# jeremiahfaith/strainer2

Measured on AMD Instinct MI355X. Metric: metagenome bases/sec scanned at k=31, higher is better.
Workload: dtype u64

## Files before the change

strainer2_amd/csrc/sk_dev_kernels.hip.h:

```cpp

__constant__ signed char sk_comp_dev[256];

struct sk_wide_view {
    const char     *keys31;
    const uint32_t *rows;
    const uint32_t *index;
    uint32_t        wmask;
    uint32_t        nwide;
};

template <bool TALLY, bool UNION = false>
__global__ __launch_bounds__(256)
void sk_scan_wide(const uint8_t *__restrict__ stream, uint64_t nbytes, uint64_t emit_begin,
                  sk_table_view table, sk_wide_view wide, sk_sink sink,
                  const uint32_t *__restrict__ flags, uint32_t *__restrict__ next_flags)
{
    if (blockIdx.x == 0u && threadIdx.x < 4u) next_flags[threadIdx.x] = 0u;
    if (flags[0] == 0u) return;
    const uint32_t nodd = flags[2];
    const bool listed = nodd <= table.oddcap;
    const uint64_t nitems = listed ? (uint64_t)nodd * 46u : nbytes;
    const uint64_t stride = (uint64_t)gridDim.x * blockDim.x;
    for (uint64_t item = (uint64_t)blockIdx.x * blockDim.x + threadIdx.x; item < nitems; item += stride) {
        uint64_t p, owner = ~0ull;
        if (listed) { owner = table.oddlist[item / 46u]; p = owner * 16u + item % 46u; }
        else p = item;
        if (p < emit_begin || p >= nbytes || p < (uint64_t)(SK_K - 1)) continue;
        const uint8_t *w = stream + (p - (SK_K - 1));
        char u[SK_K];
        bool hard = false, pure = true;
        int last_odd = -1;
        for (int i = 0; i < SK_K; i++) {
            const uint32_t b = w[i];
            hard |= (bool)sk_is_hard_break(b);
            if (!sk_is_acgt(b)) { pure = false; last_odd = i; }
            u[i] = (char)sk_upper(b);
        }
        if (hard || pure) continue;
        if (listed && ((p - (SK_K - 1) + (uint64_t)last_odd) >> 4) != owner) continue;
        int sign = 0;
        for (int i = 0; i < SK_K && sign == 0; i++) {
            const signed char f = (signed char)u[i];
            const signed char r = sk_comp_dev[(uint8_t)u[SK_K - 1 - i]];
            sign = (f > r) - (r > f);
        }
        char o[SK_K + 1];
        if (sign >= 0) { for (int i = 0; i < SK_K; i++) o[i] = u[i]; }
        else           { for (int i = 0; i < SK_K; i++) o[SK_K - 1 - i] = (char)sk_comp_dev[(uint8_t)u[i]]; }
        o[SK_K] = 0;
        bool opure = true, has_n = false, has_nul = false;
        for (int i = 0; i < SK_K; i++) {
            opure &= (bool)sk_is_acgt((uint8_t)o[i]) & ((uint8_t)o[i] < 'a');
            has_n |= (o[i] == 'N');
            has_nul |= (o[i] == 0);
        }
        if (has_n || has_nul) continue;
        if (opure) {
            uint64_t key = 0;
            for (int i = 0; i < SK_K; i++) key = (key << 2) | sk_code((uint8_t)o[i]);
            sk_probe<TALLY, false, UNION>(key, table, sink, (uint32_t)p);
        } else if (wide.nwide) {
            uint32_t slot = sk_hash_wide(o) & wide.wmask;
            for (;;) {
                const uint32_t e = wide.index[slot];
                if (e == 0u) break;
                const char *cand = wide.keys31 + (size_t)(e - 1u) * 32u;
                bool same = true;
                for (int i = 0; i < SK_K; i++) same &= (cand[i] == o[i]);
                if (same) { sk_on_hit<TALLY, false, UNION>(sink, wide.rows[e - 1u], (uint32_t)p); break; }
                slot = (slot + 1u) & wide.wmask;
            }
        }
    }
}

__global__ void sk_fill64(uint64_t *p, uint64_t n, uint64_t v)
{
    const uint64_t stride = (uint64_t)gridDim.x * blockDim.x;
    for (uint64_t i = (uint64_t)blockIdx.x * blockDim.x + threadIdx.x; i < n; i += stride) p[i] = v;
}

__global__ void sk_table_insert(const uint64_t *__restrict__ in, uint32_t n, sk_u4 *slots, uint32_t mask, uint32_t *flags,
                                const uint32_t *__restrict__ perm, const uint32_t *__restrict__ locality)
{
    const uint32_t i = blockIdx.x * blockDim.x + threadIdx.x;
    if (i >= n) return;
    const uint64_t k = in[i];
    const uint32_t idx = perm ? perm[i] : i;
    if (k == SK_EMPTY64) return;
    if (k > SK_KMASK62) { atomicAdd(&flags[1], 1u); return; }
    uint32_t slot = sk_slot0(sk_khash(k), mask);
    for (;;) {
        const unsigned long long old = atomicCAS((unsigned long long *)&slots[slot],
                                                (unsigned long long)SK_EMPTY64, (unsigned long long)k);
        if (old == SK_EMPTY64) {
            ((uint32_t *)&slots[slot])[2] = idx;
            ((uint32_t *)&slots[slot])[3] = 0xFFFFFFFEu | (locality ? locality[i] >> 31 : 0u);
            return;
        }
        if (old == k) { atomicAdd(&flags[1], 1u); return; }
        slot = (slot + 1u) & mask;
    }
}

__global__ void sk_tally_compact(const uint32_t *__restrict__ tally, uint32_t nrec, uint32_t *__restrict__ out, unsigned long long *n)
{
    const uint32_t r = blockIdx.x * blockDim.x + threadIdx.x;
    const uint2 t = r < nrec ? ((const uint2 *)tally)[r] : make_uint2(0u, 0u);
    const unsigned long long m = __ballot(t.x != 0u);
    if (!m) return;
    const uint32_t lane = threadIdx.x & 63u, leader = (uint32_t)__builtin_ctzll(m);
    unsigned long long base = 0;
    if (lane == leader) base = atomicAdd(n, (unsigned long long)__popcll(m));
    base = ((unsigned long long)(uint32_t)__shfl((int)(uint32_t)(base >> 32), (int)leader) << 32) | (uint32_t)__shfl((int)(uint32_t)base, (int)leader);
    if (t.x != 0u) {
        uint32_t *o = out + 3ull * (base + (unsigned long long)__popcll(m & ((1ull << lane) - 1ull)));
        o[0] = r; o[1] = t.x; o[2] = t.y;
    }
}

__global__ void sk_inf_bitmap(const uint32_t *__restrict__ type, uint32_t n, uint32_t value, uint32_t *__restrict__ bits)
{
    const uint32_t i = blockIdx.x * blockDim.x + threadIdx.x;
    const bool is = i < n && type[i] == value;
    const unsigned long long m = __ballot(is);
    if ((threadIdx.x & 63u) == 0u && i < n + 64u) { bits[2u * (i >> 6)] = (uint32_t)m; bits[2u * (i >> 6) + 1u] = (uint32_t)(m >> 32); }
}

__global__ void sk_table_setpos(sk_u4 *slots, uint64_t nslots, const uint32_t *__restrict__ pos_by_idx)
{
    const uint64_t stride = (uint64_t)gridDim.x * blockDim.x;
    for (uint64_t i = (uint64_t)blockIdx.x * blockDim.x + threadIdx.x; i < nslots; i += stride) {
        const sk_u4 e = slots[i];
        if (sk_slot_key(e) == SK_EMPTY64) continue;
        ((uint32_t *)&slots[i])[3] = (pos_by_idx[e.z] << 1) | (e.w & 1u);
    }
}

#define SK_DIFF_PER_BLOCK 4096u
__global__ __launch_bounds__(256) void sk_diff_block_sums(const uint32_t *__restrict__ diff, uint32_t n, uint32_t *__restrict__ sums)
{
    __shared__ uint32_t part[256];
    const uint32_t base = blockIdx.x * SK_DIFF_PER_BLOCK + threadIdx.x * 16u;
    uint32_t t = 0;
    for (uint32_t i = 0; i < 16u; i++) if (base + i < n) t += diff[base + i];
    part[threadIdx.x] = t;
    __syncthreads();
    for (uint32_t d = 128u; d > 0u; d >>= 1) { if (threadIdx.x < d) part[threadIdx.x] += part[threadIdx.x + d]; __syncthreads(); }
    if (threadIdx.x == 0) sums[blockIdx.x] = part[0];
}
__global__ __launch_bounds__(1024) void sk_diff_scan_sums(uint32_t *sums, uint32_t nb)
{
    __shared__ uint32_t part[1024];
    const uint32_t per = (nb + 1023u) / 1024u, lo = threadIdx.x * per;
    uint32_t t = 0;
    for (uint32_t i = lo; i < lo + per && i < nb; i++) t += sums[i];
    part[threadIdx.x] = t;
    __syncthreads();
    for (uint32_t d = 1u; d < 1024u; d <<= 1) {
        const uint32_t v = threadIdx.x >= d ? part[threadIdx.x - d] : 0u;
        __syncthreads();
        part[threadIdx.x] += v;
        __syncthreads();
    }
    uint32_t run = part[threadIdx.x] - t;
    for (uint32_t i = lo; i < lo + per && i < nb; i++) { const uint32_t v = sums[i]; sums[i] = run; run += v; }
}
__global__ __launch_bounds__(256) void sk_diff_apply(uint32_t *__restrict__ diff, uint32_t n, const uint32_t *__restrict__ sums,
                                                      uint32_t *__restrict__ counts, uint32_t nrows)
{
    __shared__ uint32_t part[256];
    const uint32_t base = blockIdx.x * SK_DIFF_PER_BLOCK + threadIdx.x * 16u;
    uint32_t v[16], t = 0;
    for (uint32_t i = 0; i < 16u; i++) { v[i] = base + i < n ? diff[base + i] : 0u; t += v[i]; }
    part[threadIdx.x] = t;
    __syncthreads();
    for (uint32_t d = 1u; d < 256u; d <<= 1) {
        const uint32_t u = threadIdx.x >= d ? part[threadIdx.x - d] : 0u;
        __syncthreads();
        part[threadIdx.x] += u;
        __syncthreads();
    }
    uint32_t run = sums[blockIdx.x] + part[threadIdx.x] - t;
    for (uint32_t i = 0; i < 16u; i++) {
        run += v[i];
        if (base + i < nrows && run) counts[base + i] += run;
        if (base + i < n && v[i]) diff[base + i] = 0u;
    }
}

__global__ void sk_gather_u32(uint32_t *__restrict__ dst, const uint32_t *__restrict__ src, const uint32_t *__restrict__ perm, uint32_t n)
{
    const uint32_t i = blockIdx.x * blockDim.x + threadIdx.x;
    if (i < n) dst[i] = src[perm[i]];
}

__global__ void sk_scatter_u32(uint32_t *__restrict__ dst, const uint32_t *__restrict__ src, const uint32_t *__restrict__ perm, uint32_t n)
{
    const uint32_t i = blockIdx.x * blockDim.x + threadIdx.x;
    if (i < n) dst[perm[i]] = src[i];
}

__global__ void sk_perm_from_locality(uint32_t *__restrict__ perm, const uint32_t *__restrict__ locality, uint32_t n)
{
    const uint32_t i = blockIdx.x * blockDim.x + threadIdx.x;
    if (i < n) perm[i] = locality[i] & 0x7FFFFFFFu;
}

__global__ void sk_invert_perm(uint32_t *__restrict__ inv, const uint32_t *__restrict__ perm, uint32_t n, uint32_t *flags)
{
    const uint32_t i = blockIdx.x * blockDim.x + threadIdx.x;
    if (i >= n) return;
    if (perm[i] >= n) { atomicAdd(&flags[1], 1u); return; }
    inv[perm[i]] = i;
}

__global__ void sk_grid_insert(const uint64_t *__restrict__ in, uint32_t n, uint32_t *__restrict__ w1, uint32_t nblocks1,
                               uint32_t *__restrict__ w2, uint32_t shift2)
{
    const uint32_t i = blockIdx.x * blockDim.x + threadIdx.x;
    if (i >= n) return;
    const uint64_t k = in[i];
    if (k == SK_EMPTY64) return;
    for (int off = 0; off < 16; off++) {
        const uint32_t f = (uint32_t)(k >> (2 * (15 - off)));
        const uint32_t r = sk_revcomp16(f);
        const uint32_t g = sk_gmix(f < r ? f : r);
        const uint32_t a = sk_grid1_bits(g);
        uint32_t *blk = w1 + 2u * (size_t)sk_grid1_block(g, nblocks1);
        const uint32_t m0 = (1u << ((a >> 24) & 31u)) | (1u << ((a >> 16) & 31u)), m1 = (1u << ((a >> 8) & 31u)) | (1u << (a & 31u));
        if ((__builtin_nontemporal_load(&blk[0]) & m0) != m0) atomicOr(&blk[0], m0);
        if ((__builtin_nontemporal_load(&blk[1]) & m1) != m1) atomicOr(&blk[1], m1);
    }
    for (int off = 0; off < 8; off++) sk_grid2_insert24(w2, shift2, (k >> (2 * (7 - off))) & 0xFFFFFFFFFFFFull);
}

__device__ __forceinline__ bool sk_bit(const uint32_t *__restrict__ bits, uint32_t p) { return (bits[p >> 5] >> (p & 31u)) & 1u; }
__device__ __forceinline__ uint64_t sk_text_canon(const uint32_t *__restrict__ text2, uint32_t p, uint32_t *is_fwd)
{
    const uint64_t fwd = sk_text_key(text2, p);
    uint64_t r = ((uint64_t)__builtin_bitreverse32((uint32_t)fwd) << 32) | __builtin_bitreverse32((uint32_t)(fwd >> 32));
    r = ((r >> 1) & 0x5555555555555555ull) | ((r & 0x5555555555555555ull) << 1);
    const uint64_t rc = (~r) >> 2;
    *is_fwd = fwd > rc;
    return fwd > rc ? fwd : rc;
}
__global__ void sk_build_insert(const uint32_t *__restrict__ text2, const uint32_t *__restrict__ startok, uint32_t nbases, sk_u4 *slots, uint32_t mask)
{
    const uint32_t p = blockIdx.x * blockDim.x + threadIdx.x;
    if (p + SK_K > nbases || !sk_bit(startok, p)) return;
    uint32_t fw;
    const uint64_t k = sk_text_canon(text2, p, &fw);
    uint32_t slot = sk_slot0(sk_khash(k), mask);
    for (;;) {
        const unsigned long long old = atomicCAS((unsigned long long *)&slots[slot], (unsigned long long)SK_EMPTY64, (unsigned long long)k);
        if (old == SK_EMPTY64 || old == k) { atomicMin(&((uint32_t *)&slots[slot])[3], (p << 1) | fw); return; }
        slot = (slot + 1u) & mask;
    }
}
__device__ __forceinline__ uint32_t sk_build_find(const sk_u4 *slots, uint32_t mask, uint64_t k)
{
    uint32_t slot = sk_slot0(sk_khash(k), mask);
    while (sk_slot_key(slots[slot]) != k) slot = (slot + 1u) & mask;
    return slot;
}
__global__ void sk_build_first(const uint32_t *__restrict__ text2, const uint32_t *__restrict__ startok, uint32_t nbases, const sk_u4 *slots, uint32_t mask, sk_u4 *rank)
{
    const uint32_t p = blockIdx.x * blockDim.x + threadIdx.x;
    if (p + SK_K > nbases || !sk_bit(startok, p)) return;
    uint32_t fw;
    const uint64_t k = sk_text_canon(text2, p, &fw);
    if ((slots[sk_build_find(slots, mask, k)].w >> 1) != p) return;
    atomicOr((uint32_t *)&rank[p >> 6] + ((p & 32u) ? 2 : 1), 1u << (p & 31u));
}
__global__ __launch_bounds__(1024) void sk_build_rank_scan(sk_u4 *rank, uint32_t nblk, uint32_t *total)
{
    __shared__ uint32_t part[1024];
    const uint32_t per = (nblk + 1023u) / 1024u, lo = threadIdx.x * per;
    uint32_t t = 0;
    for (uint32_t i = lo; i < lo + per && i < nblk; i++) t += (uint32_t)__popc(rank[i].y) + (uint32_t)__popc(rank[i].z);
    part[threadIdx.x] = t;
    __syncthreads();
    for (uint32_t d = 1u; d < 1024u; d <<= 1) {
        const uint32_t v = threadIdx.x >= d ? part[threadIdx.x - d] : 0u;
        __syncthreads();
        part[threadIdx.x] += v;
        __syncthreads();
    }
    uint32_t run = part[threadIdx.x] - t;
    for (uint32_t i = lo; i < lo + per && i < nblk; i++) { const uint32_t v = (uint32_t)__popc(rank[i].y) + (uint32_t)__popc(rank[i].z); rank[i].x = run; run += v; }
    if (threadIdx.x == 1023u) *total = part[1023];
}
__global__ void sk_build_index(const uint32_t *__restrict__ text2, uint32_t nbases, sk_u4 *slots, uint32_t mask, const sk_u4 *__restrict__ rank, uint64_t *__restrict__ keys_by_row)
{
    const uint32_t p = blockIdx.x * blockDim.x + threadIdx.x;
    if (p + SK_K > nbases) return;
    const sk_u4 r = rank[p >> 6];
    const uint64_t bits = ((uint64_t)r.z << 32) | r.y;
    if (!((bits >> (p & 63u)) & 1ull)) return;
    const uint32_t idx = r.x + (uint32_t)__popcll(bits & ((1ull << (p & 63u)) - 1ull));
    uint32_t fw;
    const uint64_t k = sk_text_canon(text2, p, &fw);
    ((uint32_t *)&slots[sk_build_find(slots, mask, k)])[2] = idx;
    keys_by_row[idx] = k;
}
__global__ void sk_set_rows_u32(uint32_t *__restrict__ dst, const uint32_t *__restrict__ rows, uint32_t n, const uint32_t *__restrict__ perm, uint32_t v)
{
    const uint32_t i = blockIdx.x * blockDim.x + threadIdx.x;
    if (i < n) dst[perm ? perm[rows[i]] : rows[i]] = v;
}
__global__ void sk_gather_keys(uint64_t *__restrict__ out, const uint64_t *__restrict__ keys_by_row, const uint32_t *__restrict__ rows, uint32_t n)
{
    const uint32_t i = blockIdx.x * blockDim.x + threadIdx.x;
    if (i < n) out[i] = keys_by_row[rows[i]];
}
__global__ void sk_fill32(uint32_t *p, uint32_t n, uint32_t v)
{
    const uint32_t i = blockIdx.x * blockDim.x + threadIdx.x;
    if (i < n) p[i] = v;
}

__global__ void sk_grid_insert_slots(const sk_u4 *__restrict__ slots, uint64_t nslots, uint32_t *__restrict__ w1, uint32_t nblocks1,
                                     uint32_t *__restrict__ w2, uint32_t shift2)
{
    const uint64_t stride = (uint64_t)gridDim.x * blockDim.x;
    for (uint64_t i = (uint64_t)blockIdx.x * blockDim.x + threadIdx.x; i < nslots; i += stride) {
        const uint64_t k = sk_slot_key(slots[i]);
        if (k == SK_EMPTY64) continue;
        for (int off = 0; off < 16; off++) {
            const uint32_t f = (uint32_t)(k >> (2 * (15 - off)));
            const uint32_t r = sk_revcomp16(f);
            const uint32_t g = sk_gmix(f < r ? f : r);
            const uint32_t a = sk_grid1_bits(g);
            uint32_t *blk = w1 + 2u * (size_t)sk_grid1_block(g, nblocks1);
            const uint32_t m0 = (1u << ((a >> 24) & 31u)) | (1u << ((a >> 16) & 31u)), m1 = (1u << ((a >> 8) & 31u)) | (1u << (a & 31u));
            if ((__builtin_nontemporal_load(&blk[0]) & m0) != m0) atomicOr(&blk[0], m0);
            if ((__builtin_nontemporal_load(&blk[1]) & m1) != m1) atomicOr(&blk[1], m1);
        }
        for (int off = 0; off < 8; off++) sk_grid2_insert24(w2, shift2, (k >> (2 * (7 - off))) & 0xFFFFFFFFFFFFull);
    }
}

__global__ void sk_grid_insert_text(const uint32_t *__restrict__ text2, uint32_t nbases, uint32_t *__restrict__ w1, uint32_t nblocks1,
                                    uint32_t *__restrict__ w2, uint32_t shift2)
{
    const uint32_t q = blockIdx.x * blockDim.x + threadIdx.x;
    if (q + 16u > nbases) return;
    const uint32_t w = q >> 4, o2 = 2u * (q & 15u);
    const uint32_t f = (uint32_t)(((((uint64_t)text2[w] << 32) | text2[w + 1u]) << o2) >> 32);
    const uint32_t r = sk_revcomp16(f);
    const uint32_t g = sk_gmix(f < r ? f : r);
    const uint32_t a = sk_grid1_bits(g);
    uint32_t *blk = w1 + 2u * (size_t)sk_grid1_block(g, nblocks1);
    const uint32_t m0 = (1u << ((a >> 24) & 31u)) | (1u << ((a >> 16) & 31u)), m1 = (1u << ((a >> 8) & 31u)) | (1u << (a & 31u));
    if ((__builtin_nontemporal_load(&blk[0]) & m0) != m0) atomicOr(&blk[0], m0);
    if ((__builtin_nontemporal_load(&blk[1]) & m1) != m1) atomicOr(&blk[1], m1);
    if (q + 24u <= nbases) sk_grid2_insert24(w2, shift2, sk_text_24(text2, q));
}
```

strainer2_amd/csrc/sk_device.hip:

```cpp
#include <hip/hip_runtime.h>
#include <dlfcn.h>
#include <stdarg.h>
#include <stdio.h>
#include <stdlib.h>
#include <string.h>
#include <new>
#include <string>
#include <vector>
#include <unistd.h>
#include <pthread.h>
#include <errno.h>
#include <time.h>

#include "../../include/strainer_kmer.h"
#include "sk_rendezvous.h"
#include "sk_common.h"
#include "sk_internal.h"

#include "sk_dev_scan.hip.h"
#include "sk_dev_pipeline.hip.h"
#include "sk_dev_kernels.hip.h"

#define SK_STAGE_BYTES   (64ull << 20)
#define SK_NSTAGE        2

struct sk_pin { void *p; size_t n; bool used; bool registered; };

struct sk_ctx {
    int          device;
    hipStream_t  stream;
    std::vector<sk_pin> pins;
    pthread_mutex_t pin_mu;
    sk_u4       *d_keys;
    uint32_t     slots_log2;
    uint32_t    *d_text2;
    sk_u4       *d_rank;
    uint32_t     text_bases;
    uint2       *d_grid1, *d_grid2;
    uint32_t     grid1_blocks, grid2_blocks_log2;
    long         grid_kib;
    uint64_t    *d_keys_by_row;
    bool         grid_pending;
    bool         all_rows_in_text;
    long         odd_cap;
    uint32_t     nrows, ncols;
    uint32_t    *d_counts;
    uint32_t    *d_perm, *d_inv;
    uint32_t    *d_locality;
    uint32_t    *d_tmp;
    uint32_t    *d_infbits;
    uint32_t     infbits_col, infbits_val; bool infbits_ok;
    uint32_t    *d_diff, *d_diff_sums;
    int          diff_col;
    std::vector<uint32_t> h_perm;
    char        *d_wide_keys;
    uint32_t    *d_wide_rows;
    uint32_t    *d_wide_index;
    uint32_t     wide_mask, nwide;
    uint8_t     *h_stage[SK_NSTAGE];
    uint8_t     *d_stage[SK_NSTAGE];
    hipEvent_t   stage_done[SK_NSTAGE];
    int          stage_next;
    hipStream_t  copy_stream;
    hipEvent_t   copied[64];
    hipEvent_t   read_done;
    uint64_t     tickets;
    uint32_t    *d_flags;
    uint32_t     flag_set;
    bool         flags_ready;
    uint32_t    *d_oddlist;
    std::vector<hipEvent_t> ev;
    std::vector<hipEvent_t> ev_free;
    double       timed_ms;
    uint64_t     timed_launches;
    long         table_load_pct;
    long         ablate;
    long         dev_uncached;
    uint32_t    *d_grid3;
    void        *p_bins, *p_binn, *p_cand;
    size_t       p_bins_cap, p_binn_cap, p_cand_cap;
    long         pipeline;
    long         no_text;
    void        *t_tally, *t_hits, *t_compact;
    size_t       t_tally_cap, t_hits_cap, t_compact_cap;
    uint8_t     *h_tally;
    size_t       h_tally_cap;
    uint32_t     t_inflight_nrec;
    uint64_t     t_inflight_cap;
    struct sk_batch *own_batch;
    void        *comm;
    int          comm_rank, comm_world;
    char         err[512];
};

static int sk_fail(sk_ctx *c, int code, const char *fmt, ...)
{
    if (c) {
        va_list ap;
        va_start(ap, fmt);
        vsnprintf(c->err, sizeof c->err, fmt, ap);
        va_end(ap);
    }
    return code;
}

#define SK_HIP(ctx, call)                                                                        \
    do {                                                                                         \
        hipError_t e_ = (call);                                                                  \
        if (e_ != hipSuccess)                                                                    \
            return sk_fail((ctx), SK_E_HIP, "%s failed: %s (%s:%d)", #call, hipGetErrorString(e_), \
                           __FILE__, __LINE__);                                                  \
    } while (0)

extern "C" const char *sk_strerror(int code)
{
    switch (code) {
    case SK_OK: return "ok";
    case SK_E_NODEVICE: return "no usable HIP device (this library has no CPU fallback)";
    case SK_E_HIP: return "HIP runtime error";
    case SK_E_ARG: return "bad argument";
    case SK_E_NOMEM: return "out of memory";
    case SK_E_OPEN: return "could not open file";
    case SK_E_DUPKEY: return "duplicate or malformed key in table load";
    case SK_E_STATE: return "call out of order";
    case SK_E_RCCL: return "RCCL error";
    case SK_E_SPLIT: return "a file could not be cut at record boundaries";
    case SK_E_PLAN: return "the ranks computed different work plans";
    default: return "unknown error";
    }
}

extern "C" const char *sk_last_error(const sk_ctx *ctx) { return ctx ? ctx->err : "no context"; }

extern "C" int sk_ctx_create(sk_ctx **out, int device)
{
    if (!out) return SK_E_ARG;
    *out = NULL;
    int ndev = 0;
    if (hipGetDeviceCount(&ndev) != hipSuccess || ndev <= 0) return SK_E_NODEVICE;
    if (device < 0 || device >= ndev) return SK_E_ARG;
    if (hipSetDevice(device) != hipSuccess) return SK_E_NODEVICE;
    {
        const char *e = getenv("SK_SYNC");
        if (e && !strcmp(e, "blocking")) (void)hipSetDeviceFlags(hipDeviceScheduleBlockingSync);
        else if (e && !strcmp(e, "yield")) (void)hipSetDeviceFlags(hipDeviceScheduleYield);
    }
    sk_ctx *c = new (std::nothrow) sk_ctx();
    if (!c) return SK_E_NOMEM;
    c->device = device;
    pthread_mutex_init(&c->pin_mu, NULL);
    c->table_load_pct = 50;
    c->grid_kib = -1;
    c->diff_col = -1;
    c->err[0] = 0;
    if (hipStreamCreateWithFlags(&c->stream, hipStreamNonBlocking) != hipSuccess) { delete c; return SK_E_NODEVICE; }
    if (hipMalloc((void **)&c->d_flags, 32 * sizeof(uint32_t)) != hipSuccess) { delete c; return SK_E_NOMEM; }
    if (hipMalloc((void **)&c->d_oddlist, (size_t)SK_ODDCAP * sizeof(uint32_t)) != hipSuccess) { hipFree(c->d_flags); delete c; return SK_E_NOMEM; }
    hipMemsetAsync(c->d_flags, 0, 32 * sizeof(uint32_t), c->stream);
    {
        static pthread_mutex_t once_mu = PTHREAD_MUTEX_INITIALIZER;
        static unsigned long long done_mask[4];
        pthread_mutex_lock(&once_mu);
        const bool have = device < 256 && ((done_mask[device >> 6] >> (device & 63)) & 1ull);
        hipError_t e = hipSuccess;
        if (!have) {
            signed char comp[256];
            sk_fill_complement(comp);
            e = hipMemcpyToSymbol(HIP_SYMBOL(sk_comp_dev), comp, sizeof comp);
            if (e == hipSuccess && device < 256) done_mask[device >> 6] |= 1ull << (device & 63);
        }
        pthread_mutex_unlock(&once_mu);
        if (e != hipSuccess) { delete c; return SK_E_NODEVICE; }
    }
    *out = c;
    return SK_OK;
}

static void sk_table_release(sk_ctx *c)
{
    hipFree(c->d_keys); c->d_keys = NULL;
    hipFree(c->d_text2); c->d_text2 = NULL;
    hipFree(c->d_rank); c->d_rank = NULL;
    c->text_bases = 0;
    hipFree(c->d_grid1); c->d_grid1 = NULL;
    hipFree(c->d_grid2); c->d_grid2 = NULL;
    hipFree(c->d_grid3); c->d_grid3 = NULL;
    hipFree(c->d_keys_by_row); c->d_keys_by_row = NULL;
    c->grid_pending = false; c->all_rows_in_text = false;
    hipFree(c->d_counts); c->d_counts = NULL;
    hipFree(c->d_perm); c->d_perm = NULL;
    c->h_perm.clear();
    hipFree(c->d_inv); c->d_inv = NULL;
    hipFree(c->d_locality); c->d_locality = NULL;
    hipFree(c->d_tmp); c->d_tmp = NULL;
    hipFree(c->d_diff); c->d_diff = NULL;
    hipFree(c->d_diff_sums); c->d_diff_sums = NULL;
    c->diff_col = -1;
    hipFree(c->d_infbits); c->d_infbits = NULL; c->infbits_ok = false;
    hipFree(c->d_wide_keys); c->d_wide_keys = NULL;
    hipFree(c->d_wide_rows); c->d_wide_rows = NULL;
    hipFree(c->d_wide_index); c->d_wide_index = NULL;
    c->nrows = c->ncols = c->nwide = 0;
}

extern "C" void sk_comm_destroy(sk_ctx *c);
extern "C" void sk_batch_destroy(struct sk_batch *b);

extern "C" void sk_ctx_destroy(sk_ctx *c)
{
    if (!c) return;
    hipSetDevice(c->device);
    hipStreamSynchronize(c->stream);
    sk_comm_destroy(c);
    sk_table_release(c);
    for (int i = 0; i < SK_NSTAGE; i++) {
        if (c->h_stage[i]) hipHostFree(c->h_stage[i]);
        if (c->d_stage[i]) hipFree(c->d_stage[i]);
        if (c->stage_done[i]) hipEventDestroy(c->stage_done[i]);
    }
    if (c->copy_stream) { hipStreamSynchronize(c->copy_stream); hipStreamDestroy(c->copy_stream); }
    for (hipEvent_t e : c->ev) hipEventDestroy(e);
    for (hipEvent_t e : c->ev_free) hipEventDestroy(e);
    for (int i = 0; i < 64; i++) if (c->copied[i]) hipEventDestroy(c->copied[i]);
    if (c->read_done) hipEventDestroy(c->read_done);
    if (c->own_batch) sk_batch_destroy(c->own_batch);
    hipFree(c->t_tally); hipFree(c->t_hits); hipFree(c->t_compact);
    hipFree(c->p_bins); hipFree(c->p_binn); hipFree(c->p_cand);
    if (c->h_tally) hipHostFree(c->h_tally);
    for (sk_pin &q : c->pins) { if (q.registered) { hipHostUnregister(q.p); free(q.p); } else hipHostFree(q.p); }
    pthread_mutex_destroy(&c->pin_mu);
    hipFree(c->d_flags);
    hipFree(c->d_oddlist);
    hipStreamDestroy(c->stream);
    delete c;
}

extern "C" int sk_set_option(sk_ctx *c, const char *name, long value)
{
    if (!c || !name) return SK_E_ARG;
    if (!strcmp(name, "table_load_pct")) { if (value < 5 || value > 90) return SK_E_ARG; c->table_load_pct = value; return SK_OK; }
    if (!strcmp(name, "grid_kib")) { if (value < -1 || value == 0 || value > (1 << 22)) return SK_E_ARG; c->grid_kib = value; return SK_OK; }
    if (!strcmp(name, "odd_list_cap")) { if (value < 0 || value > (long)SK_ODDCAP) return SK_E_ARG; c->odd_cap = value; return SK_OK; }
    if (!strcmp(name, "dev_alloc_uncached")) { c->dev_uncached = value != 0; return SK_OK; }
    if (!strcmp(name, "text_stage")) { c->no_text = value == 0; return SK_OK; }
    if (!strcmp(name, "pipeline")) { if (value < 0 || value > 2) return SK_E_ARG; c->pipeline = value; return SK_OK; }
#ifdef SK_EXPERIMENTS
    if (!strcmp(name, "ablate")) { c->ablate = value; return SK_OK; }
#else
    if (!strcmp(name, "ablate")) return value == 0 ? SK_OK : sk_fail(c, SK_E_ARG, "option \"ablate\" needs a library built with make EXPERIMENTS=1");
#endif
    return sk_fail(c, SK_E_ARG, "unknown option %s", name);
}

extern "C" int sk_table_load(sk_ctx *c, const uint64_t *keys, uint32_t nrows, uint32_t ncols)
{
    return sk_table_load_ex(c, keys, nrows, ncols, NULL);
}

extern "C" int sk_table_load_ex(sk_ctx *c, const uint64_t *keys, uint32_t nrows, uint32_t ncols, const uint32_t *locality)
{
    if (!c || (!keys && nrows) || ncols == 0 || ncols > 16) return SK_E_ARG;
    if (locality) {
        std::vector<uint8_t> seen(nrows, 0);
        for (uint32_t i = 0; i < nrows; i++) {
            const uint32_t l = locality[i] & 0x7FFFFFFFu;
            if (l >= nrows || seen[l]) return sk_fail(c, SK_E_ARG, "locality is not a permutation");
            seen[l] = 1;
        }
    }
    SK_HIP(c, hipSetDevice(c->device));
    SK_HIP(c, hipStreamSynchronize(c->stream));
    sk_table_release(c);

    uint32_t lg = 10;
    while (((uint64_t)1 << lg) * (uint64_t)c->table_load_pct < (uint64_t)nrows * 100ull && lg < 31) lg++;
    const uint64_t slots = (uint64_t)1 << lg;
    c->slots_log2 = lg;
    SK_HIP(c, hipMalloc((void **)&c->d_keys, slots * sizeof(sk_u4)));
    const size_t cbytes = (size_t)(nrows ? nrows : 1) * ncols * sizeof(uint32_t);
    SK_HIP(c, hipMalloc((void **)&c->d_counts, cbytes));
    SK_HIP(c, hipMemsetAsync(c->d_counts, 0, cbytes, c->stream));
    hipLaunchKernelGGL(sk_fill64, dim3(2048), dim3(256), 0, c->stream, (uint64_t *)c->d_keys, 2 * slots, SK_EMPTY64);
    SK_HIP(c, hipMemsetAsync(c->d_flags, 0, 16 * sizeof(uint32_t), c->stream));
    c->flags_ready = false;
    if (nrows) {
        uint64_t *d_in = NULL;
        SK_HIP(c, hipMalloc((void **)&d_in, (size_t)nrows * sizeof(uint64_t)));
        SK_HIP(c, hipMemcpyAsync(d_in, keys, (size_t)nrows * sizeof(uint64_t), hipMemcpyHostToDevice, c->stream));
        if (locality) {
            SK_HIP(c, hipMalloc((void **)&c->d_perm, (size_t)nrows * 4));
            SK_HIP(c, hipMalloc((void **)&c->d_inv, (size_t)nrows * 4));
            SK_HIP(c, hipMalloc((void **)&c->d_tmp, (size_t)nrows * 4));
            c->h_perm.resize(nrows);
            for (uint32_t i = 0; i < nrows; i++) c->h_perm[i] = locality[i] & 0x7FFFFFFFu;
            SK_HIP(c, hipMalloc((void **)&c->d_locality, (size_t)nrows * 4));
            SK_HIP(c, hipMemcpyAsync(c->d_locality, locality, (size_t)nrows * 4, hipMemcpyHostToDevice, c->stream));
            hipLaunchKernelGGL(sk_perm_from_locality, dim3((nrows + 255) / 256), dim3(256), 0, c->stream, c->d_perm, (const uint32_t *)c->d_locality, nrows);
            SK_HIP(c, hipMemsetAsync(c->d_inv, 0xFF, (size_t)nrows * 4, c->stream));
            hipLaunchKernelGGL(sk_invert_perm, dim3((nrows + 255) / 256), dim3(256), 0, c->stream, c->d_inv, c->d_perm, nrows, c->d_flags);
        }
        hipLaunchKernelGGL(sk_table_insert, dim3((nrows + 255) / 256), dim3(256), 0, c->stream,
                           d_in, nrows, c->d_keys, (uint32_t)(slots - 1), c->d_flags, c->d_perm, c->d_locality);
        {
            uint64_t kib = c->grid_kib > 0 ? (uint64_t)c->grid_kib : ((uint64_t)nrows * 23ull / 32ull + 1023ull) / 1024ull;
            if (kib > (1ull << 22)) kib = 1ull << 22;
            if (kib < 4ull) kib = 4ull;
            c->grid1_blocks = (uint32_t)(kib * 1024ull / sizeof(uint2));
            uint32_t g2 = 12;
            while (g2 < 34 && ((uint64_t)1 << g2) < (uint64_t)nrows * 32ull) g2++;
            c->grid2_blocks_log2 = g2 - 6u;
            const size_t b1 = (size_t)c->grid1_blocks * sizeof(uint2), b2 = ((size_t)1 << c->grid2_blocks_log2) * sizeof(uint2);
            SK_HIP(c, hipMalloc((void **)&c->d_grid1, b1));
            SK_HIP(c, hipMalloc((void **)&c->d_grid2, b2));
            SK_HIP(c, hipMemsetAsync(c->d_grid1, 0, b1, c->stream));
            SK_HIP(c, hipMemsetAsync(c->d_grid2, 0, b2, c->stream));
            c->grid_pending = true;
            c->all_rows_in_text = false;
        }
        uint32_t flags[2] = {0, 0};
        SK_HIP(c, hipMemcpyAsync(flags, c->d_flags, sizeof flags, hipMemcpyDeviceToHost, c->stream));
        SK_HIP(c, hipStreamSynchronize(c->stream));
        hipFree(d_in);
        if (flags[1]) { sk_table_release(c); return sk_fail(c, SK_E_DUPKEY, "%u duplicate/malformed keys", flags[1]); }
    }
    SK_HIP(c, hipGetLastError());
    c->nrows = nrows;
    c->ncols = ncols;
    return SK_OK;
}

extern "C" int sk_table_load_wide(sk_ctx *c, const char *keys31, const uint32_t *rows, uint32_t nwide)
{
    if (!c) return SK_E_ARG;
    if (!c->d_keys) return sk_fail(c, SK_E_STATE, "sk_table_load first");
    if (nwide == 0) return SK_OK;
    if (!keys31 || !rows) return SK_E_ARG;
    SK_HIP(c, hipSetDevice(c->device));
    uint32_t lg = 4;
    while (((uint32_t)1 << lg) < nwide * 2u) lg++;
    const uint32_t wslots = (uint32_t)1 << lg;
    std::vector<uint32_t> index(wslots, 0u);
    for (uint32_t i = 0; i < nwide; i++) {
        if (rows[i] >= c->nrows) return sk_fail(c, SK_E_ARG, "wide row %u out of range", rows[i]);
        uint32_t slot = sk_hash_wide(keys31 + (size_t)i * 32) & (wslots - 1);
        while (index[slot]) slot = (slot + 1) & (wslots - 1);
        index[slot] = i + 1;
    }
    SK_HIP(c, hipMalloc((void **)&c->d_wide_keys, (size_t)nwide * 32));
    SK_HIP(c, hipMalloc((void **)&c->d_wide_rows, (size_t)nwide * sizeof(uint32_t)));
    SK_HIP(c, hipMalloc((void **)&c->d_wide_index, (size_t)wslots * sizeof(uint32_t)));
    SK_HIP(c, hipMemcpy(c->d_wide_keys, keys31, (size_t)nwide * 32, hipMemcpyHostToDevice));
    std::vector<uint32_t> wrows(rows, rows + nwide);
    if (!c->h_perm.empty()) for (uint32_t i = 0; i < nwide; i++) wrows[i] = c->h_perm[rows[i]];
    SK_HIP(c, hipMemcpy(c->d_wide_rows, wrows.data(), (size_t)nwide * sizeof(uint32_t), hipMemcpyHostToDevice));
    SK_HIP(c, hipMemcpy(c->d_wide_index, index.data(), (size_t)wslots * sizeof(uint32_t), hipMemcpyHostToDevice));
    c->wide_mask = wslots - 1;
    c->nwide = nwide;
    return SK_OK;
}

extern "C" int sk_table_load_text(sk_ctx *c, const uint32_t *text2, uint32_t nbases, const uint32_t *first_pos)
{
    if (!c || !text2 || !first_pos) return SK_E_ARG;
    if (!c->d_keys || !c->nrows) return sk_fail(c, SK_E_STATE, "sk_table_load_ex first");
    if (c->h_perm.empty()) return sk_fail(c, SK_E_STATE, "the text stage needs the locality order of sk_table_load_ex");
    if (nbases < SK_K || nbases > 0x7FFFFF00u) return sk_fail(c, SK_E_ARG, "text of %u bases (a table slot holds 31 bits of position)", nbases);
    const uint32_t nrows = c->nrows;
    std::vector<uint32_t> pos_by_idx(nrows, 0xFFFFFFFFu);
    for (uint32_t r = 0; r < nrows; r++) pos_by_idx[c->h_perm[r]] = first_pos[r];
    uint32_t m = 0;
    while (m < nrows && pos_by_idx[m] != 0xFFFFFFFFu) m++;
    for (uint32_t i = 0; i < nrows; i++) {
        const uint32_t p = pos_by_idx[i];
        if (i >= m) { if (p != 0xFFFFFFFFu) return sk_fail(c, SK_E_ARG, "rows with a text position must come first in locality order"); continue; }
        if (p > nbases - SK_K || (i && p <= pos_by_idx[i - 1])) return sk_fail(c, SK_E_ARG, "text positions must ascend with the locality order and lie inside the text");
    }
    const size_t nblk = (size_t)nbases / 64 + 2;
    std::vector<sk_u4> rank(nblk, (sk_u4){0u, 0u, 0u, 0u});
    for (uint32_t i = 0; i < m; i++) {
        const uint32_t p = pos_by_idx[i];
        if (p & 32u) rank[p >> 6].z |= 1u << (p & 31u); else rank[p >> 6].y |= 1u << (p & 31u);
    }
    uint32_t run = 0;
    for (size_t b = 0; b < nblk; b++) { rank[b].x = run; run += (uint32_t)__builtin_popcount(rank[b].y) + (uint32_t)__builtin_popcount(rank[b].z); }
    SK_HIP(c, hipSetDevice(c->device));
    SK_HIP(c, hipStreamSynchronize(c->stream));
    hipFree(c->d_text2); c->d_text2 = NULL;
    hipFree(c->d_rank); c->d_rank = NULL;
    c->text_bases = 0;
    const size_t words = (size_t)nbases / 16 + 4, have = ((size_t)nbases + 15) / 16;
    SK_HIP(c, hipMalloc((void **)&c->d_text2, words * 4));
    SK_HIP(c, hipMalloc((void **)&c->d_rank, nblk * sizeof(sk_u4)));
    hipFree(c->d_diff); c->d_diff = NULL;
    hipFree(c->d_diff_sums); c->d_diff_sums = NULL;
    c->diff_col = -1;
    SK_HIP(c, hipMalloc((void **)&c->d_diff, ((size_t)nrows + 2) * 4));
    SK_HIP(c, hipMalloc((void **)&c->d_diff_sums, ((size_t)nrows / SK_DIFF_PER_BLOCK + 2) * 4));
    SK_HIP(c, hipMemsetAsync(c->d_diff, 0, ((size_t)nrows + 2) * 4, c->stream));
    SK_HIP(c, hipMemsetAsync(c->d_text2, 0, words * 4, c->stream));
    SK_HIP(c, hipMemcpyAsync(c->d_text2, text2, have * 4, hipMemcpyHostToDevice, c->stream));
    SK_HIP(c, hipMemcpyAsync(c->d_rank, rank.data(), nblk * sizeof(sk_u4), hipMemcpyHostToDevice, c->stream));
    SK_HIP(c, hipMemcpyAsync(c->d_tmp, pos_by_idx.data(), (size_t)nrows * 4, hipMemcpyHostToDevice, c->stream));
    hipLaunchKernelGGL(sk_table_setpos, dim3(4096), dim3(256), 0, c->stream, c->d_keys, (uint64_t)1 << c->slots_log2, c->d_tmp);
    c->all_rows_in_text = m == nrows;
    if (c->grid_pending && c->all_rows_in_text) {
        hipLaunchKernelGGL(sk_grid_insert_text, dim3((nbases + 255) / 256), dim3(256), 0, c->stream, (const uint32_t *)c->d_text2, nbases,
                           (uint32_t *)c->d_grid1, c->grid1_blocks, (uint32_t *)c->d_grid2, 32u - c->grid2_blocks_log2);
        c->grid_pending = false;
    }
    SK_HIP(c, hipStreamSynchronize(c->stream));
    SK_HIP(c, hipGetLastError());
    c->text_bases = nbases;
    return SK_OK;
}

static int sk_table_build_from_text_steps(sk_ctx *c, const uint32_t *text2, const uint32_t *startok, uint32_t nbases, uint32_t nstarts,
                                          uint32_t ncols, uint32_t col0_value, uint32_t *nrows_out, uint32_t *&d_ok);
extern "C" int sk_table_build_from_text(sk_ctx *c, const uint32_t *text2, const uint32_t *startok, uint32_t nbases, uint32_t nstarts,
                                        uint32_t ncols, uint32_t col0_value, uint32_t *nrows_out)
{
    if (!c || !text2 || !startok || !nrows_out || ncols == 0 || ncols > 16) return SK_E_ARG;
    if (nbases < SK_K || nbases > 0x7FFFFF00u) return sk_fail(c, SK_E_ARG, "text of %u bases (a table slot holds 31 bits of position)", nbases);
    SK_HIP(c, hipSetDevice(c->device));
    SK_HIP(c, hipStreamSynchronize(c->stream));
    sk_table_release(c);
    uint32_t *d_ok = NULL;
    const int rc = sk_table_build_from_text_steps(c, text2, startok, nbases, nstarts, ncols, col0_value, nrows_out, d_ok);
    if (d_ok) (void)hipFree(d_ok);
    if (rc != SK_OK) {
        (void)hipStreamSynchronize(c->stream);
        sk_table_release(c);
        c->nrows = 0; c->ncols = 0;
    }
    return rc;
}

static int sk_table_build_from_text_steps(sk_ctx *c, const uint32_t *text2, const uint32_t *startok, uint32_t nbases, uint32_t nstarts,
                                          uint32_t ncols, uint32_t col0_value, uint32_t *nrows_out, uint32_t *&d_ok)
{
    uint32_t lg = 10;
    while (((uint64_t)1 << lg) * (uint64_t)c->table_load_pct < (uint64_t)nstarts * 100ull && lg < 31) lg++;
    const uint64_t slots = (uint64_t)1 << lg;
    const uint32_t mask = (uint32_t)(slots - 1);
    c->slots_log2 = lg;
    const size_t words = (size_t)nbases / 16 + 4, have = ((size_t)nbases + 15) / 16, nblk = (size_t)nbases / 64 + 2, bwords = ((size_t)nbases + 31) / 32;
    uint32_t *d_total = NULL;
    SK_HIP(c, hipMalloc((void **)&c->d_keys, slots * sizeof(sk_u4)));
    SK_HIP(c, hipMalloc((void **)&c->d_text2, words * 4));
    SK_HIP(c, hipMalloc((void **)&c->d_rank, nblk * sizeof(sk_u4)));
    SK_HIP(c, hipMalloc((void **)&d_ok, bwords * 4 + 4));
    d_total = d_ok + bwords;
    hipLaunchKernelGGL(sk_fill64, dim3(2048), dim3(256), 0, c->stream, (uint64_t *)c->d_keys, 2 * slots, SK_EMPTY64);
    SK_HIP(c, hipMemsetAsync(c->d_text2, 0, words * 4, c->stream));
    SK_HIP(c, hipMemsetAsync(c->d_rank, 0, nblk * sizeof(sk_u4), c->stream));
    SK_HIP(c, hipMemsetAsync(c->d_flags, 0, 16 * sizeof(uint32_t), c->stream));
    c->flags_ready = false;
    SK_HIP(c, hipMemcpyAsync(c->d_text2, text2, have * 4, hipMemcpyHostToDevice, c->stream));
    SK_HIP(c, hipMemcpyAsync(d_ok, startok, bwords * 4, hipMemcpyHostToDevice, c->stream));
    const dim3 grid((nbases + 255) / 256), block(256);
    hipLaunchKernelGGL(sk_build_insert, grid, block, 0, c->stream, (const uint32_t *)c->d_text2, (const uint32_t *)d_ok, nbases, c->d_keys, mask);
    hipLaunchKernelGGL(sk_build_first, grid, block, 0, c->stream, (const uint32_t *)c->d_text2, (const uint32_t *)d_ok, nbases, (const sk_u4 *)c->d_keys, mask, c->d_rank);
    hipLaunchKernelGGL(sk_build_rank_scan, dim3(1), dim3(1024), 0, c->stream, c->d_rank, (uint32_t)nblk, d_total);
    uint32_t nrows = 0;
    SK_HIP(c, hipMemcpyAsync(&nrows, d_total, 4, hipMemcpyDeviceToHost, c->stream));
    SK_HIP(c, hipStreamSynchronize(c->stream));
    (void)hipFree(d_ok);
    d_ok = NULL;
    *nrows_out = nrows;
    c->nrows = nrows; c->ncols = ncols;
    c->text_bases = nbases;
    c->all_rows_in_text = true;
    const size_t cbytes = (size_t)(nrows ? nrows : 1) * ncols * sizeof(uint32_t);
    SK_HIP(c, hipMalloc((void **)&c->d_counts, cbytes));
    SK_HIP(c, hipMemsetAsync(c->d_counts, 0, cbytes, c->stream));
    if (nrows) {
        SK_HIP(c, hipMalloc((void **)&c->d_keys_by_row, (size_t)nrows * 8));
        hipLaunchKernelGGL(sk_build_index, grid, block, 0, c->stream, (const uint32_t *)c->d_text2, nbases, c->d_keys, mask, (const sk_u4 *)c->d_rank, c->d_keys_by_row);
        if (col0_value) hipLaunchKernelGGL(sk_fill32, dim3((nrows + 255) / 256), dim3(256), 0, c->stream, c->d_counts, nrows, col0_value);
        uint64_t kib = c->grid_kib > 0 ? (uint64_t)c->grid_kib : ((uint64_t)nrows * 23ull / 32ull + 1023ull) / 1024ull;
        if (kib > (1ull << 22)) kib = 1ull << 22;
        if (kib < 4ull) kib = 4ull;
        c->grid1_blocks = (uint32_t)(kib * 1024ull / sizeof(uint2));
        uint32_t g2 = 12;
        while (g2 < 34 && ((uint64_t)1 << g2) < (uint64_t)nrows * 32ull) g2++;
        c->grid2_blocks_log2 = g2 - 6u;
        const size_t b1 = (size_t)c->grid1_blocks * sizeof(uint2), b2 = ((size_t)1 << c->grid2_blocks_log2) * sizeof(uint2);
        SK_HIP(c, hipMalloc((void **)&c->d_grid1, b1));
        SK_HIP(c, hipMalloc((void **)&c->d_grid2, b2));
        SK_HIP(c, hipMemsetAsync(c->d_grid1, 0, b1, c->stream));
        SK_HIP(c, hipMemsetAsync(c->d_grid2, 0, b2, c->stream));
        hipLaunchKernelGGL(sk_grid_insert_text, grid, block, 0, c->stream, (const uint32_t *)c->d_text2, nbases,
                           (uint32_t *)c->d_grid1, c->grid1_blocks, (uint32_t *)c->d_grid2, 32u - c->grid2_blocks_log2);
        c->grid_pending = false;
        c->diff_col = -1;
        SK_HIP(c, hipMalloc((void **)&c->d_diff, ((size_t)nrows + 2) * 4));
        SK_HIP(c, hipMalloc((void **)&c->d_diff_sums, ((size_t)nrows / SK_DIFF_PER_BLOCK + 2) * 4));
        SK_HIP(c, hipMemsetAsync(c->d_diff, 0, ((size_t)nrows + 2) * 4, c->stream));
    } else {
        c->grid1_blocks = 512; c->grid2_blocks_log2 = 6;
        SK_HIP(c, hipMalloc((void **)&c->d_grid1, 512 * sizeof(uint2)));
        SK_HIP(c, hipMalloc((void **)&c->d_grid2, 64 * sizeof(uint2)));
        SK_HIP(c, hipMemsetAsync(c->d_grid1, 0, 512 * sizeof(uint2), c->stream));
        SK_HIP(c, hipMemsetAsync(c->d_grid2, 0, 64 * sizeof(uint2), c->stream));
    }
    SK_HIP(c, hipStreamSynchronize(c->stream));
    SK_HIP(c, hipGetLastError());
    return SK_OK;
}

extern "C" int sk_table_export_keys(sk_ctx *c, uint64_t *keys_out)
{
    if (!c || (!keys_out && c->nrows)) return SK_E_ARG;
    if (!c->d_keys_by_row && c->nrows) return sk_fail(c, SK_E_STATE, "no key list to export (sk_table_build_from_text first)");
    SK_HIP(c, hipSetDevice(c->device));
    if (c->nrows) SK_HIP(c, hipMemcpy(keys_out, c->d_keys_by_row, (size_t)c->nrows * 8, hipMemcpyDeviceToHost));
    return SK_OK;
}
extern "C" int sk_table_export_keys_of(sk_ctx *c, const uint32_t *rows, uint32_t n, uint64_t *keys_out)
{
    if (!c || (n && (!rows || !keys_out))) return SK_E_ARG;
    if (!n) return SK_OK;
    if (!c->d_keys_by_row) return sk_fail(c, SK_E_STATE, "no key list to export (sk_table_build_from_text first)");
    for (uint32_t i = 0; i < n; i++) if (rows[i] >= c->nrows) return sk_fail(c, SK_E_ARG, "row %u out of range", rows[i]);
    SK_HIP(c, hipSetDevice(c->device));
    void *d = NULL;
    SK_HIP(c, hipMalloc(&d, (size_t)n * 12));
    uint64_t *d_out = (uint64_t *)d;
    uint32_t *d_rows = (uint32_t *)(d_out + n);
    hipError_t e = hipMemcpyAsync(d_rows, rows, (size_t)n * 4, hipMemcpyHostToDevice, c->stream);
    if (e == hipSuccess) {
        hipLaunchKernelGGL(sk_gather_keys, dim3((n + 255) / 256), dim3(256), 0, c->stream, d_out, (const uint64_t *)c->d_keys_by_row, (const uint32_t *)d_rows, n);
        e = hipMemcpyAsync(keys_out, d_out, (size_t)n * 8, hipMemcpyDeviceToHost, c->stream);
    }
    if (e == hipSuccess) e = hipStreamSynchronize(c->stream);
    (void)hipFree(d);
    SK_HIP(c, e);
    return SK_OK;
}

static int sk_grid_ensure(sk_ctx *c)
{
    if (!c->grid_pending) return SK_OK;
    hipLaunchKernelGGL(sk_grid_insert_slots, dim3(4096), dim3(256), 0, c->stream, (const sk_u4 *)c->d_keys, (uint64_t)1 << c->slots_log2,
                       (uint32_t *)c->d_grid1, c->grid1_blocks, (uint32_t *)c->d_grid2, 32u - c->grid2_blocks_log2);
    SK_HIP(c, hipGetLastError());
    c->grid_pending = false;
    return SK_OK;
}

static int sk_diff_flush(sk_ctx *c)
{
    if (c->diff_col < 0 || !c->d_diff) { c->diff_col = -1; return SK_OK; }
    const uint32_t n = c->nrows + 1u, nb = (n + SK_DIFF_PER_BLOCK - 1u) / SK_DIFF_PER_BLOCK;
    hipLaunchKernelGGL(sk_diff_block_sums, dim3(nb), dim3(256), 0, c->stream, c->d_diff, n, c->d_diff_sums);
    hipLaunchKernelGGL(sk_diff_scan_sums, dim3(1), dim3(1024), 0, c->stream, c->d_diff_sums, nb);
    hipLaunchKernelGGL(sk_diff_apply, dim3(nb), dim3(256), 0, c->stream, c->d_diff, n, c->d_diff_sums,
                       c->d_counts + (size_t)c->diff_col * c->nrows, c->nrows);
    c->diff_col = -1;
    SK_HIP(c, hipGetLastError());
    return SK_OK;
}

static int sk_scratch(sk_ctx *c, void **p, size_t *cap, size_t need);

static int sk_launch_scan(sk_ctx *c, const uint8_t *d_stream, uint64_t nbytes, uint64_t emit_begin, uint32_t col,
                          const sk_sink *tally_sink = NULL, const void *packed_inv = NULL)
{
    if (nbytes <= emit_begin || c->nrows == 0) return SK_OK;
    const uint64_t ntiles = (nbytes + SK_TILE - 1) / SK_TILE;
    if (ntiles > 0x7FFFFFFFull) return sk_fail(c, SK_E_ARG, "batch too large");
    sk_table_view tv;
    tv.nrows = c->nrows;
    tv.text2 = c->no_text ? NULL : c->d_text2; tv.rank = c->d_rank; tv.text_bases = c->text_bases;
    tv.slots = c->d_keys; tv.mask = (uint32_t)(((uint64_t)1 << c->slots_log2) - 1);
    tv.oddlist = c->d_oddlist; tv.oddcap = c->odd_cap ? (uint32_t)c->odd_cap : SK_ODDCAP;
    tv.grid1 = c->d_grid1; tv.grid2 = c->d_grid2;
    tv.grid1_blocks = c->grid1_blocks; tv.grid2_shift = 32u - c->grid2_blocks_log2;
    sk_wide_view wv;
    wv.keys31 = c->d_wide_keys; wv.rows = c->d_wide_rows; wv.index = c->d_wide_index;
    wv.wmask = c->wide_mask; wv.nwide = c->nwide;
    sk_sink sink;
    memset(&sink, 0, sizeof sink);
    if (tally_sink) sink = *tally_sink;
    else {
        c->infbits_ok = false;
        sink.counts = c->d_counts + (size_t)col * c->nrows;
        sink.diff = c->d_diff;
        if (tv.text2 && c->diff_col != (int)col) {
            int rc = sk_diff_flush(c);
            if (rc) return rc;
            c->diff_col = (int)col;
        }
    }
    const dim3 grid((uint32_t)ntiles), block(SK_THREADS);
    if (!c->d_grid1) return sk_fail(c, SK_E_STATE, "no table loaded");
    { int grc = sk_grid_ensure(c); if (grc) return grc; }

    if (!c->flags_ready) {
        SK_HIP(c, hipMemsetAsync(c->d_flags, 0, 8 * sizeof(uint32_t), c->stream));
        c->flags_ready = true;
    }
    c->flag_set ^= 1u;
    uint32_t *const d_fl = c->d_flags + 4u * c->flag_set, *const d_fl_next = c->d_flags + 4u * (c->flag_set ^ 1u);
    hipEvent_t e0 = NULL, e1 = NULL;
    const bool timed = true;
    if (c->ev.size() >= 2 * SK_EV_PAIRS) {
        float ms = 0.f;
        SK_HIP(c, hipEventSynchronize(c->ev[1]));
        SK_HIP(c, hipEventElapsedTime(&ms, c->ev[0], c->ev[1]));
        c->timed_ms += ms;
        c->timed_launches++;
        c->ev_free.push_back(c->ev[0]);
        c->ev_free.push_back(c->ev[1]);
        c->ev.erase(c->ev.begin(), c->ev.begin() + 2);
    }
    if (c->ev_free.size() >= 2) {
        e1 = c->ev_free.back(); c->ev_free.pop_back();
        e0 = c->ev_free.back(); c->ev_free.pop_back();
    } else {
        SK_HIP(c, hipEventCreate(&e0));
        SK_HIP(c, hipEventCreate(&e1));
    }
    SK_HIP(c, hipEventRecord(e0, c->stream));
    const bool piped = !packed_inv && (!c->ablate || c->ablate >= 7) && c->pipeline == 2;
    const uint8_t *d_cand = NULL;
    if (piped && !c->d_grid3) {
        const size_t b3 = (size_t)SK_BIN_P * SK_BIN_WORDS * 4;
        const uint64_t nslots = (uint64_t)1 << c->slots_log2;
        SK_HIP(c, hipMalloc((void **)&c->d_grid3, b3));
        SK_HIP(c, hipMemsetAsync(c->d_grid3, 0, b3, c->stream));
        hipLaunchKernelGGL(sk_grid3_insert, dim3((uint32_t)((nslots + 255) / 256)), dim3(256), 0, c->stream, (const sk_u4 *)c->d_keys, nslots, c->d_grid3);
    }
    if (piped) {
        const uint64_t ntiles_bin = (nbytes + SK_BIN_TILE - 1) / SK_BIN_TILE;
        int rc;
        if ((rc = sk_scratch(c, &c->p_bins, &c->p_bins_cap, (size_t)ntiles_bin * SK_BIN_P * SK_BIN_CAP * 4)) != SK_OK) return rc;
        if ((rc = sk_scratch(c, &c->p_binn, &c->p_binn_cap, (size_t)ntiles_bin * SK_BIN_P)) != SK_OK) return rc;
        if ((rc = sk_scratch(c, &c->p_cand, &c->p_cand_cap, (size_t)ntiles_bin * SK_BIN_CH + 64)) != SK_OK) return rc;
        SK_HIP(c, hipMemsetAsync(c->p_cand, 0, (size_t)ntiles_bin * SK_BIN_CH + 64, c->stream));
        hipLaunchKernelGGL(sk_bin, dim3((uint32_t)ntiles_bin), dim3(256), 0, c->stream, d_stream, nbytes, tv,
                           (uint32_t *)c->p_bins, (uint8_t *)c->p_binn, (uint32_t)ntiles_bin, (uint8_t *)c->p_cand, d_fl);
        uint32_t splits = ntiles_bin >= 4096 ? 4u : ntiles_bin >= 1024 ? 2u : 1u;
        static bool lds_attr = false;
        if (!lds_attr) {
            SK_HIP(c, hipFuncSetAttribute((const void *)sk_lds_probe, hipFuncAttributeMaxDynamicSharedMemorySize, (int)(SK_BIN_WORDS * 4)));
            lds_attr = true;
        }
        hipLaunchKernelGGL(sk_lds_probe, dim3(SK_BIN_P * splits), dim3(1024), SK_BIN_WORDS * 4, c->stream, (const uint32_t *)c->d_grid3,
                           (const uint32_t *)c->p_bins, (const uint8_t *)c->p_binn, (uint32_t)ntiles_bin, splits, (uint8_t *)c->p_cand);
        d_cand = (const uint8_t *)c->p_cand;
    }
#define SK_LAUNCH_GRID(T, A, C) hipLaunchKernelGGL((sk_scan_grid<T, A, C>), grid, block, 0, c->stream, \
                                                   d_stream, nbytes, emit_begin, tv, sink, d_fl, d_cand)
    if (packed_inv) {
        if (c->ablate) return sk_fail(c, SK_E_UNSUPPORTED, "no ablations on packed batches");
        if (tally_sink && tally_sink->ns)
            hipLaunchKernelGGL((sk_scan_grid<true, 0, false, true, true>), grid, block, 0, c->stream, d_stream, nbytes, emit_begin, tv, sink, d_fl, (const uint8_t *)packed_inv);
        else if (tally_sink)
            hipLaunchKernelGGL((sk_scan_grid<true, 0, false, false, true>), grid, block, 0, c->stream, d_stream, nbytes, emit_begin, tv, sink, d_fl, (const uint8_t *)packed_inv);
        else
            hipLaunchKernelGGL((sk_scan_grid<false, 0, false, false, true>), grid, block, 0, c->stream, d_stream, nbytes, emit_begin, tv, sink, d_fl, (const uint8_t *)packed_inv);
    }
    else if (tally_sink && tally_sink->ns)
        hipLaunchKernelGGL((sk_scan_grid<true, 0, false, true>), grid, block, 0, c->stream, d_stream, nbytes, emit_begin, tv, sink, d_fl, d_cand);
    else if (piped && tally_sink) SK_LAUNCH_GRID(true, 0, true);
#ifdef SK_EXPERIMENTS
    else if (piped && c->ablate == 7) SK_LAUNCH_GRID(false, 7, true);
    else if (piped && c->ablate == 8) SK_LAUNCH_GRID(false, 8, true);
    else if (piped && c->ablate == 9) SK_LAUNCH_GRID(false, 9, true);
#endif
    else if (piped)          SK_LAUNCH_GRID(false, 0, true);
    else if (tally_sink)     SK_LAUNCH_GRID(true, 0, false);
#ifdef SK_EXPERIMENTS
    else if (c->ablate == 1) SK_LAUNCH_GRID(false, 1, false);
    else if (c->ablate == 2) SK_LAUNCH_GRID(false, 2, false);
    else if (c->ablate == 3) SK_LAUNCH_GRID(false, 3, false);
    else if (c->ablate == 4) SK_LAUNCH_GRID(false, 4, false);
    else if (c->ablate == 5) SK_LAUNCH_GRID(false, 5, false);
    else if (c->ablate == 6) SK_LAUNCH_GRID(false, 6, false);
    else if (c->ablate == 10) SK_LAUNCH_GRID(false, 10, false);
#endif
    else                     SK_LAUNCH_GRID(false, 0, false);
#undef SK_LAUNCH_GRID
    if (timed) {
        SK_HIP(c, hipEventRecord(e1, c->stream));
        c->ev.push_back(e0);
        c->ev.push_back(e1);
    }
    uint64_t wblocks = (nbytes - emit_begin + 255) / 256;
    if (wblocks > 2048) wblocks = 2048;
    if (wblocks == 0) { wblocks = 1; }
    if (tally_sink && tally_sink->ns)
        hipLaunchKernelGGL((sk_scan_wide<true, true>), dim3((uint32_t)wblocks), dim3(256), 0, c->stream,
                           d_stream, nbytes, emit_begin, tv, wv, sink, d_fl, d_fl_next);
    else if (tally_sink)
        hipLaunchKernelGGL(sk_scan_wide<true>, dim3((uint32_t)wblocks), dim3(256), 0, c->stream,
                           d_stream, nbytes, emit_begin, tv, wv, sink, d_fl, d_fl_next);
    else
        hipLaunchKernelGGL(sk_scan_wide<false>, dim3((uint32_t)wblocks), dim3(256), 0, c->stream,
                           d_stream, nbytes, emit_begin, tv, wv, sink, d_fl, d_fl_next);
    SK_HIP(c, hipGetLastError());
    return SK_OK;
}

static int sk_scratch(sk_ctx *c, void **p, size_t *cap, size_t need)
{
    if (need <= *cap) return SK_OK;
    if (*p) { SK_HIP(c, hipStreamSynchronize(c->stream)); (void)hipFree(*p); *p = NULL; *cap = 0; }
    size_t want = need + need / 4 + 4096;
    SK_HIP(c, hipMalloc(p, want));
    *cap = want;
    return SK_OK;
}

struct sk_batch {
    sk_ctx      *owner;
    hipStream_t  stream;
    hipEvent_t   ready;
    void        *d_stream, *d_rec;
    size_t       stream_cap, rec_cap;
    uint64_t     nbytes;
    uint32_t     nrec, ntiles;
    bool         packed;
    uint32_t    *h_rec;
    size_t       h_rec_cap;
};

extern "C" int sk_batch_create(sk_ctx *c, sk_batch **out)
{
    if (!c || !out) return SK_E_ARG;
    *out = NULL;
    SK_HIP(c, hipSetDevice(c->device));
    sk_batch *b = new (std::nothrow) sk_batch();
    if (!b) return SK_E_NOMEM;
    b->owner = c;
    b->d_stream = b->d_rec = NULL; b->stream_cap = b->rec_cap = 0; b->nbytes = 0; b->nrec = b->ntiles = 0;
    b->h_rec = NULL; b->h_rec_cap = 0; b->packed = false;
    if (hipStreamCreateWithFlags(&b->stream, hipStreamNonBlocking) != hipSuccess) { delete b; return sk_fail(c, SK_E_HIP, "stream"); }
    if (hipEventCreateWithFlags(&b->ready, hipEventDisableTiming) != hipSuccess) { hipStreamDestroy(b->stream); delete b; return sk_fail(c, SK_E_HIP, "event"); }
    *out = b;
    return SK_OK;
}

extern "C" int sk_batch_sync(sk_batch *b)
{
    if (!b) return SK_E_ARG;
    SK_HIP(b->owner, hipSetDevice(b->owner->device));
    SK_HIP(b->owner, hipStreamSynchronize(b->stream));
    return SK_OK;
}

extern "C" void sk_batch_destroy(sk_batch *b)
{
    if (!b) return;
    hipSetDevice(b->owner->device);
    hipStreamSynchronize(b->stream);
    hipFree(b->d_stream); hipFree(b->d_rec);
    if (b->h_rec) hipHostFree(b->h_rec);
    hipEventDestroy(b->ready);
    hipStreamDestroy(b->stream);
    delete b;
}

static int sk_batch_fill_any(sk_batch *b, const uint8_t *stream, uint64_t nbytes, const uint32_t *rec_start, uint32_t nrec, bool packed);
extern "C" int sk_batch_fill(sk_batch *b, const uint8_t *stream, uint64_t nbytes, const uint32_t *rec_start, uint32_t nrec)
{
    return sk_batch_fill_any(b, stream, nbytes, rec_start, nrec, false);
}
extern "C" int sk_batch_fill_packed(sk_batch *b, const void *packed, uint64_t nbytes, const uint32_t *rec_start, uint32_t nrec)
{
    return sk_batch_fill_any(b, (const uint8_t *)packed, nbytes, rec_start, nrec, true);
}
static int sk_batch_fill_any(sk_batch *b, const uint8_t *stream, uint64_t nbytes, const uint32_t *rec_start, uint32_t nrec, bool packed)
{
    if (!b || !stream || !rec_start) return SK_E_ARG;
    sk_ctx *c = b->owner;
    if (nbytes == 0 || nrec == 0 || nbytes > 0xFFFFFFF0ull) return sk_fail(c, SK_E_ARG, "bad batch size");
    SK_HIP(c, hipSetDevice(c->device));
    const uint32_t ntiles = (uint32_t)((nbytes + 32767u) >> 15);
    if (nbytes + 16 > b->stream_cap) {
        SK_HIP(c, hipStreamSynchronize(b->stream));
        (void)hipFree(b->d_stream); b->d_stream = NULL; b->stream_cap = 0;
        const size_t want = nbytes + nbytes / 4 + 4096;
        SK_HIP(c, hipMalloc(&b->d_stream, want));
        b->stream_cap = want;
    }
    const size_t rec_need = ((size_t)nrec + ntiles + 2) * 4;
    if (rec_need > b->rec_cap) {
        SK_HIP(c, hipStreamSynchronize(b->stream));
        (void)hipFree(b->d_rec); b->d_rec = NULL; b->rec_cap = 0;
        const size_t want = rec_need + rec_need / 4 + 4096;
        SK_HIP(c, hipMalloc(&b->d_rec, want));
        b->rec_cap = want;
    }
    SK_HIP(c, hipStreamSynchronize(b->stream));
    if (rec_need > b->h_rec_cap) {
        if (b->h_rec) (void)hipHostFree(b->h_rec);
        b->h_rec = NULL; b->h_rec_cap = 0;
        const size_t want = rec_need + rec_need / 4 + 4096;
        SK_HIP(c, hipHostMalloc((void **)&b->h_rec, want, hipHostMallocDefault));
        b->h_rec_cap = want;
    }
    memcpy(b->h_rec, rec_start, (size_t)nrec * 4);
    uint32_t *const tile_first = b->h_rec + nrec;
    for (uint32_t t = 0, r = 0; t < ntiles + 2; t++) {
        const uint64_t edge = (uint64_t)t << 15;
        while (r < nrec && rec_start[r] < edge) r++;
        tile_first[t] = r;
    }
    SK_HIP(c, hipMemcpyAsync(b->d_stream, stream, packed ? ((nbytes + 15u) >> 4) * 6u : nbytes, hipMemcpyHostToDevice, b->stream));
    b->packed = packed;
    SK_HIP(c, hipMemcpyAsync(b->d_rec, b->h_rec, ((size_t)nrec + ntiles + 2) * 4, hipMemcpyHostToDevice, b->stream));
    SK_HIP(c, hipEventRecord(b->ready, b->stream));
    b->nbytes = nbytes; b->nrec = nrec; b->ntiles = ntiles;
    return SK_OK;
}

extern "C" int sk_tally_launch(sk_ctx *c, const sk_batch *b, uint32_t type_col, uint32_t informative_value, uint64_t hits_cap)
{
    if (!c || !b) return SK_E_ARG;
    if (!c->d_keys) return sk_fail(c, SK_E_STATE, "no table loaded");
    if (type_col >= c->ncols) return sk_fail(c, SK_E_ARG, "column %u out of range", type_col);
    if (b->owner->device != c->device) return sk_fail(c, SK_E_ARG, "batch lives on another device");
    if (b->nrec == 0) return sk_fail(c, SK_E_STATE, "empty batch");
    SK_HIP(c, hipSetDevice(c->device));
    int rc;
    if ((rc = sk_diff_flush(c)) != SK_OK) return rc;
    const uint32_t nrec = b->nrec;
    if ((rc = sk_scratch(c, &c->t_tally, &c->t_tally_cap, (size_t)nrec * 8 + 16)) != SK_OK) return rc;
    if ((rc = sk_scratch(c, &c->t_compact, &c->t_compact_cap, (size_t)nrec * 12 + 16)) != SK_OK) return rc;
    if ((rc = sk_scratch(c, &c->t_hits, &c->t_hits_cap, (size_t)(hits_cap ? hits_cap : 1) * sizeof(uint2))) != SK_OK) return rc;
    if ((size_t)nrec * 8 + 16 > c->h_tally_cap) {
        if (c->h_tally) { SK_HIP(c, hipStreamSynchronize(c->stream)); (void)hipHostFree(c->h_tally); c->h_tally = NULL; c->h_tally_cap = 0; }
        const size_t want = (size_t)nrec * 10 + 4096;
        SK_HIP(c, hipHostMalloc((void **)&c->h_tally, want, hipHostMallocDefault));
        c->h_tally_cap = want;
    }
    unsigned long long *d_n = (unsigned long long *)((uint8_t *)c->t_tally + (size_t)nrec * 8);
    SK_HIP(c, hipStreamWaitEvent(c->stream, b->ready, 0));
    SK_HIP(c, hipMemsetAsync(c->t_tally, 0, (size_t)nrec * 8 + 16, c->stream));
    sk_sink sink;
    memset(&sink, 0, sizeof sink);
    sink.rec_start = (const uint32_t *)b->d_rec; sink.nrec = nrec; sink.tally = (uint32_t *)c->t_tally;
    sink.tile_first = (const uint32_t *)b->d_rec + nrec;
    sink.type = c->d_counts + (size_t)type_col * c->nrows; sink.inf_value = informative_value;
    sink.hits = (uint2 *)c->t_hits; sink.nhits = d_n; sink.hits_cap = hits_cap; sink.inv = c->d_inv;
    if (!c->infbits_ok || c->infbits_col != type_col || c->infbits_val != informative_value) {
        if (!c->d_infbits) SK_HIP(c, hipMalloc((void **)&c->d_infbits, ((size_t)c->nrows / 32 + 8) * 4));
        SK_HIP(c, hipMemsetAsync(c->d_infbits, 0, ((size_t)c->nrows / 32 + 8) * 4, c->stream));
        hipLaunchKernelGGL(sk_inf_bitmap, dim3((c->nrows + 255) / 256), dim3(256), 0, c->stream, sink.type, c->nrows, informative_value, c->d_infbits);
        c->infbits_ok = true; c->infbits_col = type_col; c->infbits_val = informative_value;
    }
    sink.infbits = c->d_infbits;
    rc = sk_launch_scan(c, (const uint8_t *)b->d_stream, b->nbytes, 0, 0, &sink, b->packed ? (const uint8_t *)b->d_stream + ((b->nbytes + 15u) >> 4) * 4u : NULL);
    if (rc) return rc;
    hipLaunchKernelGGL(sk_tally_compact, dim3((nrec + 255) / 256), dim3(256), 0, c->stream, (const uint32_t *)c->t_tally, nrec,
                       (uint32_t *)c->t_compact, d_n + 1);
    SK_HIP(c, hipMemcpyAsync(c->h_tally, d_n, 16, hipMemcpyDeviceToHost, c->stream));
    c->t_inflight_nrec = nrec;
    c->t_inflight_cap = hits_cap;
    return SK_OK;
}

extern "C" int sk_tally_collect(sk_ctx *c, uint32_t *out_tally, sk_hit *out_hits, uint64_t *out_nhits)
{
    if (!c || !out_tally || !out_nhits) return SK_E_ARG;
    if (!c->t_inflight_nrec) return sk_fail(c, SK_E_STATE, "no tally in flight");
    SK_HIP(c, hipSetDevice(c->device));
    SK_HIP(c, hipStreamSynchronize(c->stream));
    const uint32_t nrec = c->t_inflight_nrec;
    c->t_inflight_nrec = 0;
    SK_HIP(c, hipMemcpy(out_tally, c->t_tally, (size_t)nrec * 8, hipMemcpyDeviceToHost));
    unsigned long long nh;
    memcpy(&nh, c->h_tally, 8);
    const unsigned long long take = nh < c->t_inflight_cap ? nh : c->t_inflight_cap;
    if (take && !out_hits) return SK_E_ARG;
    if (take) SK_HIP(c, hipMemcpy(out_hits, c->t_hits, (size_t)take * sizeof(uint2), hipMemcpyDeviceToHost));
    *out_nhits = nh;
    return SK_OK;
}

extern "C" int sk_tally_collect_sparse(sk_ctx *c, sk_tally_rec *out, uint64_t cap, uint64_t *n, sk_hit *out_hits, uint64_t *out_nhits)
{
    if (!c || !n || !out_nhits || (cap && !out)) return SK_E_ARG;
    if (!c->t_inflight_nrec) return sk_fail(c, SK_E_STATE, "no tally in flight");
    SK_HIP(c, hipSetDevice(c->device));
    SK_HIP(c, hipStreamSynchronize(c->stream));
    c->t_inflight_nrec = 0;
    unsigned long long two[2];
    memcpy(two, c->h_tally, 16);
    const unsigned long long take_r = two[1] < cap ? two[1] : cap;
    if (take_r) SK_HIP(c, hipMemcpy(out, c->t_compact, (size_t)take_r * sizeof(sk_tally_rec), hipMemcpyDeviceToHost));
    *n = two[1];
    const unsigned long long take = two[0] < c->t_inflight_cap ? two[0] : c->t_inflight_cap;
    if (take && !out_hits) return SK_E_ARG;
    if (take) SK_HIP(c, hipMemcpy(out_hits, c->t_hits, (size_t)take * sizeof(uint2), hipMemcpyDeviceToHost));
    *out_nhits = two[0];
    return SK_OK;
}

extern "C" int sk_tally_batch(sk_ctx *c, const uint8_t *stream, uint64_t nbytes, const uint32_t *rec_start, uint32_t nrec,
                              uint32_t type_col, uint32_t informative_value, uint32_t *out_tally,
                              sk_hit *out_hits, uint64_t hits_cap, uint64_t *out_nhits)
{
    if (!c || !stream || !rec_start || !out_tally || !out_nhits || (hits_cap && !out_hits)) return SK_E_ARG;
    if (!c->d_keys) return sk_fail(c, SK_E_STATE, "no table loaded");
    int rc;
    if (!c->own_batch && (rc = sk_batch_create(c, &c->own_batch)) != SK_OK) return rc;
    if ((rc = sk_batch_fill(c->own_batch, stream, nbytes, rec_start, nrec)) != SK_OK) return rc;
    if ((rc = sk_tally_launch(c, c->own_batch, type_col, informative_value, hits_cap)) != SK_OK) return rc;
    return sk_tally_collect(c, out_tally, out_hits, out_nhits);
}


#include "sk_dev_union.hip.h"

struct sk_union {
    sk_ctx   *uc;
    uint32_t  n;
    void     *d_tally, *d_flag, *d_raw;
    size_t    tally_cap, flag_cap, raw_cap;
    unsigned long long *d_cnt;
    uint32_t  cnt_set;
    bool      cnt_clean;
    uint64_t *d_ukeys;
    uint2    *d_umask;
    sk_union_member *d_members;
    std::vector<sk_ctx *> mem;
    std::vector<uint32_t> base;
    uint32_t *d_canon;
};

extern "C" void sk_union_destroy(sk_union *u)
{
    if (!u) return;
    if (u->uc) {
        hipSetDevice(u->uc->device);
        hipStreamSynchronize(u->uc->stream);
        hipFree(u->d_ukeys); hipFree(u->d_umask); hipFree(u->d_members);
        hipFree(u->d_tally); hipFree(u->d_flag); hipFree(u->d_raw); hipFree(u->d_cnt); hipFree(u->d_canon);
        sk_ctx_destroy(u->uc);
    }
    delete u;
}

extern "C" int sk_union_create(sk_ctx *const *members, uint32_t n, uint32_t type_col, uint32_t informative_value, sk_union **out)
{
    if (!members || !out || n < 1 || n > SK_UNION_MAX) return SK_E_ARG;
    *out = NULL;
    sk_ctx *first = members[0];
    if (!first) return SK_E_ARG;
    uint64_t rows = 0, tbases = 0;
    for (uint32_t s = 0; s < n; s++) {
        sk_ctx *m = members[s];
        if (!m) return SK_E_ARG;
        if (m->device != first->device) return sk_fail(first, SK_E_ARG, "the members of a union live on one device");
        if (!m->d_keys || !m->nrows) return sk_fail(first, SK_E_STATE, "member %u has no table", s);
        if (type_col >= m->ncols) return sk_fail(first, SK_E_ARG, "column %u out of range", type_col);
        if (m->nwide) return sk_fail(first, SK_E_STATE, "member %u has byte-string keys: no union", s);
        if (!m->d_text2 || !m->d_rank || m->no_text) return sk_fail(first, SK_E_STATE, "member %u has no text stage: no union", s);
        if (m->nrows >= (1u << SK_UNION_ROW_BITS) - 1u) return sk_fail(first, SK_E_STATE, "member %u has too many rows for the union's hit log", s);
        rows += m->nrows;
        tbases += ((uint64_t)m->text_bases + 63u) / 64u * 64u + 64u;
    }
    if (rows > 0x7FFFFFF0ull || tbases > 0x7FFFFF00ull) return sk_fail(first, SK_E_STATE, "union too large (%llu rows, %llu bases)", (unsigned long long)rows, (unsigned long long)tbases);
    SK_HIP(first, hipSetDevice(first->device));
    sk_union *u = new (std::nothrow) sk_union();
    if (!u) return SK_E_NOMEM;
    u->uc = NULL; u->n = n; u->d_ukeys = NULL; u->d_umask = NULL; u->d_members = NULL;
    u->d_tally = u->d_flag = u->d_raw = NULL; u->tally_cap = u->flag_cap = u->raw_cap = 0; u->d_cnt = NULL; u->d_canon = NULL;
    int rc = sk_ctx_create(&u->uc, first->device);
    if (rc != SK_OK) { delete u; return rc; }
    sk_ctx *c = u->uc;
#define SK_U(call) do { hipError_t e_ = (call); if (e_ != hipSuccess) { sk_fail(first, SK_E_HIP, "%s failed: %s", #call, hipGetErrorString(e_)); (void)hipGetLastError(); sk_union_destroy(u); return SK_E_HIP; } } while (0)
    const uint32_t nrows = (uint32_t)rows;
    uint32_t lg = 10;
    while (((uint64_t)1 << lg) * (uint64_t)first->table_load_pct < rows * 100ull && lg < 31) lg++;
    const uint64_t slots = (uint64_t)1 << lg;
    c->slots_log2 = lg;
    c->nrows = nrows; c->ncols = 1;
    SK_U(hipMalloc((void **)&c->d_keys, slots * sizeof(sk_u4)));
    SK_U(hipMalloc((void **)&u->d_ukeys, (size_t)nrows * 8));
    SK_U(hipMalloc((void **)&u->d_umask, (size_t)nrows * 8));
    uint32_t *d_canon = NULL;
    SK_U(hipMalloc((void **)&d_canon, (size_t)nrows * 4));
    hipLaunchKernelGGL(sk_fill64, dim3(2048), dim3(256), 0, c->stream, (uint64_t *)c->d_keys, 2 * slots, SK_EMPTY64);
    hipLaunchKernelGGL(sk_fill64, dim3(2048), dim3(256), 0, c->stream, u->d_ukeys, (uint64_t)nrows, SK_EMPTY64);
    SK_U(hipMemsetAsync(u->d_umask, 0, (size_t)nrows * 8, c->stream));
    const uint32_t text_bases = (uint32_t)tbases;
    const size_t words = (size_t)text_bases / 16 + 4, nblk = (size_t)text_bases / 64 + 2;
    SK_U(hipMalloc((void **)&c->d_text2, words * 4));
    SK_U(hipMalloc((void **)&c->d_rank, nblk * sizeof(sk_u4)));
    SK_U(hipMemsetAsync(c->d_text2, 0, words * 4, c->stream));
    std::vector<sk_union_member> hm(n);
    uint32_t base = 0, tbase = 0;
    for (uint32_t s = 0; s < n; s++) {
        sk_ctx *m = members[s];
        int frc = sk_diff_flush(m);
        if (frc != SK_OK) { hipFree(d_canon); sk_union_destroy(u); return frc; }
        SK_U(hipStreamSynchronize(m->stream));
        const uint64_t mslots = (uint64_t)1 << m->slots_log2;
        hipLaunchKernelGGL(sk_union_insert, dim3(4096), dim3(256), 0, c->stream, (const sk_u4 *)m->d_keys, mslots, base, tbase,
                           c->d_keys, (uint32_t)(slots - 1), u->d_ukeys);
        const uint32_t span = (uint32_t)(((uint64_t)m->text_bases + 63u) / 64u * 64u + 64u);
        SK_U(hipMemcpyAsync(c->d_text2 + tbase / 16u, m->d_text2, (((size_t)m->text_bases + 15) / 16) * 4, hipMemcpyDeviceToDevice, c->stream));
        const uint32_t nsrc = m->text_bases / 64u + 1u, ndst = span / 64u;
        hipLaunchKernelGGL(sk_union_rank_copy, dim3((ndst + 255) / 256), dim3(256), 0, c->stream, c->d_rank + tbase / 64u, (const sk_u4 *)m->d_rank,
                           nsrc < ndst ? nsrc : ndst, ndst, base, base + m->nrows);
        hm[s].slots = m->d_keys; hm[s].mask = (uint32_t)(mslots - 1); hm[s].inv = m->d_inv;
        u->mem.push_back(m);
        u->base.push_back(base);
        base += m->nrows;
        tbase += span;
    }
    hipLaunchKernelGGL(sk_union_rank_copy, dim3(1), dim3(256), 0, c->stream, c->d_rank + tbase / 64u, (const sk_u4 *)c->d_rank, 0u, (uint32_t)(nblk - tbase / 64u), 0u, nrows);
    base = 0;
    for (uint32_t s = 0; s < n; s++) {
        sk_ctx *m = members[s];
        hipLaunchKernelGGL(sk_union_mask_a, dim3(4096), dim3(256), 0, c->stream, (const sk_u4 *)m->d_keys, (uint64_t)1 << m->slots_log2, base, s,
                           (const uint32_t *)(m->d_counts + (size_t)type_col * m->nrows), informative_value,
                           (const sk_u4 *)c->d_keys, (uint32_t)(slots - 1), u->d_umask, d_canon);
        base += m->nrows;
    }
    hipLaunchKernelGGL(sk_union_mask_b, dim3((nrows + 255) / 256), dim3(256), 0, c->stream, u->d_umask, (const uint32_t *)d_canon, nrows);
    {
        uint64_t kib = first->grid_kib > 0 ? (uint64_t)first->grid_kib * n : ((uint64_t)nrows * 23ull / 32ull + 1023ull) / 1024ull;
        if (kib > (1ull << 22)) kib = 1ull << 22;
        if (kib < 4ull) kib = 4ull;
        c->grid1_blocks = (uint32_t)(kib * 1024ull / sizeof(uint2));
        uint32_t g2 = 12;
        while (g2 < 37 && ((uint64_t)1 << g2) < (uint64_t)nrows * 32ull) g2++;
        c->grid2_blocks_log2 = g2 - 6u;
        const size_t b1 = (size_t)c->grid1_blocks * sizeof(uint2), b2 = ((size_t)1 << c->grid2_blocks_log2) * sizeof(uint2);
        SK_U(hipMalloc((void **)&c->d_grid1, b1));
        SK_U(hipMalloc((void **)&c->d_grid2, b2));
        SK_U(hipMemsetAsync(c->d_grid1, 0, b1, c->stream));
        SK_U(hipMemsetAsync(c->d_grid2, 0, b2, c->stream));
        bool from_text = true;
        for (uint32_t s2 = 0; s2 < n; s2++) from_text = from_text && members[s2]->all_rows_in_text;
        if (from_text)
            hipLaunchKernelGGL(sk_grid_insert_text, dim3((text_bases + 255) / 256), dim3(256), 0, c->stream, (const uint32_t *)c->d_text2, text_bases,
                               (uint32_t *)c->d_grid1, c->grid1_blocks, (uint32_t *)c->d_grid2, 32u - c->grid2_blocks_log2);
        else
            hipLaunchKernelGGL(sk_grid_insert, dim3((nrows + 255) / 256), dim3(256), 0, c->stream, (const uint64_t *)u->d_ukeys, nrows,
                               (uint32_t *)c->d_grid1, c->grid1_blocks, (uint32_t *)c->d_grid2, 32u - c->grid2_blocks_log2);
    }
    SK_U(hipMalloc((void **)&u->d_members, n * sizeof(sk_union_member)));
    SK_U(hipMemcpyAsync(u->d_members, hm.data(), n * sizeof(sk_union_member), hipMemcpyHostToDevice, c->stream));
    SK_U(hipStreamSynchronize(c->stream));
    hipFree(d_canon);
    SK_U(hipGetLastError());
#undef SK_U
    c->text_bases = text_bases;
    *out = u;
    return SK_OK;
}

static int sk_union_zeroed(sk_union *u, void **p, size_t *cap, size_t need)
{
    sk_ctx *c = u->uc;
    if (need <= *cap) return SK_OK;
    if (*p) { SK_HIP(c, hipStreamSynchronize(c->stream)); (void)hipFree(*p); *p = NULL; *cap = 0; }
    const size_t want = need + need / 4 + 4096;
    SK_HIP(c, hipMalloc(p, want));
    SK_HIP(c, hipMemsetAsync(*p, 0, want, c->stream));
    *cap = want;
    return SK_OK;
}

extern "C" int sk_union_tally_launch(sk_union *u, const sk_batch *b, uint64_t hits_cap)
{
    if (!u || !b) return SK_E_ARG;
    sk_ctx *c = u->uc;
    if (b->owner->device != c->device) return sk_fail(c, SK_E_ARG, "batch lives on another device");
    if (b->nrec == 0) return sk_fail(c, SK_E_STATE, "empty batch");
    const uint64_t vrec = (uint64_t)b->nrec * u->n;
    if (vrec > 0x7FFFFFF0ull) return sk_fail(c, SK_E_ARG, "too many records x members");
    SK_HIP(c, hipSetDevice(c->device));
    int rc;
    if ((rc = sk_union_zeroed(u, &u->d_tally, &u->tally_cap, (size_t)vrec * 8 + 16)) != SK_OK) return rc;
    if ((rc = sk_union_zeroed(u, &u->d_flag, &u->flag_cap, (size_t)b->nrec + 16)) != SK_OK) return rc;
    if (!u->d_cnt) { SK_HIP(c, hipMalloc((void **)&u->d_cnt, 64)); u->cnt_clean = false; }
    if ((rc = sk_scratch(c, &u->d_raw, &u->raw_cap, (size_t)(hits_cap ? hits_cap : 1) * sizeof(uint2))) != SK_OK) return rc;
    if ((rc = sk_scratch(c, &c->t_compact, &c->t_compact_cap, (size_t)vrec * 12 + 16)) != SK_OK) return rc;
    if ((rc = sk_scratch(c, &c->t_hits, &c->t_hits_cap, (size_t)(hits_cap ? hits_cap : 1) * sizeof(uint2))) != SK_OK) return rc;
    const size_t land = 64 + (size_t)SK_UNION_EAGER * (sizeof(sk_tally_rec) + sizeof(uint2));
    if (c->h_tally_cap < land) {
        if (c->h_tally) { SK_HIP(c, hipStreamSynchronize(c->stream)); (void)hipHostFree(c->h_tally); c->h_tally = NULL; c->h_tally_cap = 0; }
        SK_HIP(c, hipHostMalloc((void **)&c->h_tally, land, hipHostMallocDefault));
        c->h_tally_cap = land;
    }
    SK_HIP(c, hipStreamWaitEvent(c->stream, b->ready, 0));
    if (!u->cnt_clean) {
        SK_HIP(c, hipMemsetAsync(u->d_cnt, 0, 64, c->stream));
        u->cnt_set = 1;
    }
    u->cnt_clean = false;
    u->cnt_set ^= 1u;
    unsigned long long *const d_cnt = u->d_cnt + 4u * u->cnt_set, *const d_cnt_next = u->d_cnt + 4u * (u->cnt_set ^ 1u);
    uint8_t *d_land = NULL;
    SK_HIP(c, hipHostGetDevicePointer((void **)&d_land, c->h_tally, 0));
    sk_sink sink;
    memset(&sink, 0, sizeof sink);
    sink.rec_start = (const uint32_t *)b->d_rec; sink.nrec = b->nrec; sink.tally = (uint32_t *)u->d_tally;
    sink.tile_first = (const uint32_t *)b->d_rec + b->nrec;
    sink.hits = (uint2 *)u->d_raw; sink.nhits = d_cnt; sink.hits_cap = hits_cap;
    sink.type = (const uint32_t *)u->d_umask; sink.ns = u->n;
    sink.infbits = (const uint32_t *)u->d_flag;
    rc = sk_launch_scan(c, (const uint8_t *)b->d_stream, b->nbytes, 0, 0, &sink, b->packed ? (const uint8_t *)b->d_stream + ((b->nbytes + 15u) >> 4) * 4u : NULL);
    if (rc) return rc;
    {
        uint32_t sets = (b->nrec + 256u * 256u - 1u) / (256u * 256u);
        if (sets < 1u) sets = 1u;
        if (sets > SK_UC_SETS_MAX) sets = SK_UC_SETS_MAX;
        const uint32_t ncompact = (b->nrec + 256u * sets - 1u) / (256u * sets);
        sk_union_resolve_args ra;
        ra.raw = (const uint2 *)u->d_raw; ra.nraw = d_cnt; ra.cap_raw = hits_cap;
        ra.out = (uint2 *)c->t_hits; ra.nout = d_cnt + 2; ra.cap_out = hits_cap;
        ra.ukeys = (const uint64_t *)u->d_ukeys; ra.umask = (const uint2 *)u->d_umask; ra.mem = (const sk_union_member *)u->d_members;
        hipLaunchKernelGGL(sk_union_post, dim3(ncompact + 256u), dim3(256), 0, c->stream, (uint2 *)u->d_tally, (uint8_t *)u->d_flag,
                           b->nrec, u->n, (uint32_t *)c->t_compact, d_cnt + 1, sets, ncompact, ra);
    }
    hipLaunchKernelGGL(sk_union_ship, dim3(32), dim3(256), 0, c->stream, (const unsigned long long *)d_cnt, d_cnt_next,
                       (const uint32_t *)c->t_compact, (unsigned long long)vrec, (const uint2 *)c->t_hits, (unsigned long long)hits_cap,
                       (uint32_t)SK_UNION_EAGER, d_land);
    SK_HIP(c, hipGetLastError());
    u->cnt_clean = true;
    c->t_inflight_nrec = (uint32_t)vrec;
    c->t_inflight_cap = hits_cap;
    return SK_OK;
}

extern "C" int sk_union_tally_collect(sk_union *u, sk_tally_rec *out, uint64_t cap, uint64_t *n, sk_hit *out_hits, uint64_t *out_nhits)
{
    if (!u || !n || !out_nhits || (cap && !out)) return SK_E_ARG;
    sk_ctx *c = u->uc;
    if (!c->t_inflight_nrec) return sk_fail(c, SK_E_STATE, "no tally in flight");
    SK_HIP(c, hipSetDevice(c->device));
    SK_HIP(c, hipStreamSynchronize(c->stream));
    c->t_inflight_nrec = 0;
    unsigned long long cnt[3];
    memcpy(cnt, c->h_tally, 24);
    const unsigned long long take_r = cnt[1] < cap ? cnt[1] : cap;
    {
        const unsigned long long have = take_r < SK_UNION_EAGER ? take_r : SK_UNION_EAGER;
        if (have) memcpy(out, c->h_tally + 64, (size_t)have * sizeof(sk_tally_rec));
        if (take_r > have) SK_HIP(c, hipMemcpy(out + have, (const sk_tally_rec *)c->t_compact + have, (size_t)(take_r - have) * sizeof(sk_tally_rec), hipMemcpyDeviceToHost));
    }
    *n = cnt[1];
    unsigned long long nh = cnt[2];
    if (cnt[0] > c->t_inflight_cap && nh <= c->t_inflight_cap) nh = cnt[0] > nh ? cnt[0] : c->t_inflight_cap + 1;
    const unsigned long long take = nh < c->t_inflight_cap ? nh : c->t_inflight_cap;
    if (take && !out_hits) return SK_E_ARG;
    {
        const unsigned long long have = take < SK_UNION_EAGER ? take : SK_UNION_EAGER;
        if (have) memcpy(out_hits, c->h_tally + 64 + (size_t)SK_UNION_EAGER * sizeof(sk_tally_rec), (size_t)have * sizeof(uint2));
        if (take > have) SK_HIP(c, hipMemcpy(out_hits + have, (const uint2 *)c->t_hits + have, (size_t)(take - have) * sizeof(uint2), hipMemcpyDeviceToHost));
    }
    *out_nhits = nh;
    return SK_OK;
}

extern "C" int sk_union_sync(sk_union *u)
{
    if (!u) return SK_E_ARG;
    sk_ctx *c = u->uc;
    SK_HIP(c, hipSetDevice(c->device));
    SK_HIP(c, hipStreamSynchronize(c->stream));
    c->t_inflight_nrec = 0;
    return SK_OK;
}

#define SK_UNION_MALLOC(ctx, call) do { hipError_t e_ = (call); if (e_ != hipSuccess) { (void)hipGetLastError(); \
    return sk_fail((ctx), SK_E_HIP, "%s failed: %s", #call, hipGetErrorString(e_)); } } while (0)
extern "C" int sk_union_count_enable(sk_union *u, uint32_t ncols)
{
    if (!u || ncols < 1 || ncols > 16) return SK_E_ARG;
    sk_ctx *c = u->uc;
    if (c->d_counts) return ncols == c->ncols ? SK_OK : sk_fail(c, SK_E_STATE, "the union already has %u count column(s)", c->ncols);
    SK_HIP(c, hipSetDevice(c->device));
    const uint32_t nrows = c->nrows;
    const uint64_t uslots = (uint64_t)1 << c->slots_log2;
    SK_UNION_MALLOC(c, hipMalloc((void **)&u->d_canon, (size_t)nrows * 4));
    for (uint32_t s = 0; s < u->n; s++) {
        const sk_ctx *m = u->mem[s];
        hipLaunchKernelGGL(sk_union_canon_rows, dim3(4096), dim3(256), 0, c->stream, (const sk_u4 *)m->d_keys, (uint64_t)1 << m->slots_log2,
                           u->base[s], (const sk_u4 *)c->d_keys, (uint32_t)(uslots - 1), u->d_canon);
    }
    const size_t cbytes = (size_t)nrows * ncols * 4;
    SK_UNION_MALLOC(c, hipMalloc((void **)&c->d_counts, cbytes));
    SK_HIP(c, hipMemsetAsync(c->d_counts, 0, cbytes, c->stream));
    SK_UNION_MALLOC(c, hipMalloc((void **)&c->d_diff, ((size_t)nrows + 2) * 4));
    SK_UNION_MALLOC(c, hipMalloc((void **)&c->d_diff_sums, ((size_t)nrows / SK_DIFF_PER_BLOCK + 2) * 4));
    SK_HIP(c, hipMemsetAsync(c->d_diff, 0, ((size_t)nrows + 2) * 4, c->stream));
    c->diff_col = -1;
    c->ncols = ncols;
    SK_HIP(c, hipGetLastError());
    SK_HIP(c, hipStreamSynchronize(c->stream));
    return SK_OK;
}

extern "C" sk_ctx *sk_union_context(sk_union *u) { return u ? u->uc : NULL; }

extern "C" int sk_union_counts_fold(sk_union *u, uint32_t ucol, uint32_t member_col, uint32_t member_mask, int subtract)
{
    if (!u) return SK_E_ARG;
    sk_ctx *c = u->uc;
    if (!c->d_counts || !u->d_canon) return sk_fail(c, SK_E_STATE, "the union has no count columns (sk_union_count_enable)");
    if (ucol >= c->ncols) return sk_fail(c, SK_E_ARG, "union column %u out of range", ucol);
    if (u->n < 32u && (member_mask >> u->n) != 0u) return sk_fail(c, SK_E_ARG, "member mask 0x%x names no member of %u", member_mask, u->n);
    for (uint32_t s = 0; s < u->n; s++)
        if (((member_mask >> s) & 1u) && (!u->mem[s]->d_counts || member_col >= u->mem[s]->ncols))
            return sk_fail(c, SK_E_ARG, "member %u has no column %u", s, member_col);
    SK_HIP(c, hipSetDevice(c->device));
    { int rc = sk_diff_flush(c); if (rc) return rc; }
    const uint32_t nrows = c->nrows;
    uint32_t *const uc = c->d_counts + (size_t)ucol * nrows;
    if (nrows) hipLaunchKernelGGL(sk_union_fold_canon, dim3((nrows + 255) / 256), dim3(256), 0, c->stream, uc, (const uint32_t *)u->d_canon, nrows);
    for (uint32_t s = 0; s < u->n; s++) {
        if (!((member_mask >> s) & 1u)) continue;
        sk_ctx *m = u->mem[s];
        { int rc = sk_diff_flush(m); if (rc) return rc; }
        SK_HIP(c, hipStreamSynchronize(m->stream));
        m->infbits_ok = false;
        if (m->nrows)
            hipLaunchKernelGGL(sk_union_fold_member, dim3((m->nrows + 255) / 256), dim3(256), 0, c->stream, m->d_counts + (size_t)member_col * m->nrows,
                               (const uint32_t *)uc, (const uint32_t *)u->d_canon, u->base[s], m->nrows, (uint32_t)(subtract != 0));
    }
    SK_HIP(c, hipMemsetAsync(uc, 0, (size_t)nrows * 4, c->stream));
    SK_HIP(c, hipGetLastError());
    SK_HIP(c, hipStreamSynchronize(c->stream));
    return SK_OK;
}

extern "C" int sk_union_scan_timing(sk_union *u, double *total_ms, uint64_t *launches, int reset)
{
    return u ? sk_scan_timing(u->uc, total_ms, launches, reset) : SK_E_ARG;
}
extern "C" const char *sk_union_last_error(const sk_union *u) { return u ? u->uc->err : "no union"; }
extern "C" uint32_t sk_union_members(const sk_union *u) { return u ? u->n : 0u; }
extern "C" uint32_t sk_union_rows(const sk_union *u) { return u ? u->uc->nrows : 0u; }

extern "C" int sk_scan_device(sk_ctx *c, const void *dev_stream, uint64_t nbytes, uint32_t col)
{
    if (!c || (!dev_stream && nbytes)) return SK_E_ARG;
    if (!c->d_keys) return sk_fail(c, SK_E_STATE, "no table loaded");
    if (!c->d_counts) return sk_fail(c, SK_E_STATE, "no count columns (a union's context needs sk_union_count_enable)");
    if (col >= c->ncols) return sk_fail(c, SK_E_ARG, "column %u out of range", col);
    if (((uintptr_t)dev_stream & 15u) != 0) return sk_fail(c, SK_E_ARG, "device stream must be 16-byte aligned");
    SK_HIP(c, hipSetDevice(c->device));
    return sk_launch_scan(c, (const uint8_t *)dev_stream, nbytes, 0, col);
}

extern "C" int sk_scan_device_packed(sk_ctx *c, const void *dev_packed, uint64_t nbytes, uint32_t col)
{
    if (!c || (!dev_packed && nbytes)) return SK_E_ARG;
    if (!c->d_keys) return sk_fail(c, SK_E_STATE, "no table loaded");
    if (!c->d_counts) return sk_fail(c, SK_E_STATE, "no count columns (a union's context needs sk_union_count_enable)");
    if (col >= c->ncols) return sk_fail(c, SK_E_ARG, "column %u out of range", col);
    if (((uintptr_t)dev_packed & 3u) != 0) return sk_fail(c, SK_E_ARG, "device batch must be 4-byte aligned");
    SK_HIP(c, hipSetDevice(c->device));
    const uint64_t nch = (nbytes + 15u) >> 4;
    return sk_launch_scan(c, (const uint8_t *)dev_packed, nbytes, 0, col, NULL, (const uint8_t *)dev_packed + nch * 4u);
}

static int sk_stage_init(sk_ctx *c)
{
    if (c->h_stage[0]) return SK_OK;
    for (int i = 0; i < SK_NSTAGE; i++) {
        SK_HIP(c, hipHostMalloc((void **)&c->h_stage[i], SK_STAGE_BYTES, hipHostMallocDefault));
        SK_HIP(c, hipMalloc((void **)&c->d_stage[i], SK_STAGE_BYTES));
        SK_HIP(c, hipEventCreateWithFlags(&c->stage_done[i], hipEventDisableTiming));
    }
    SK_HIP(c, hipStreamCreateWithFlags(&c->copy_stream, hipStreamNonBlocking));
    return SK_OK;
}

extern "C" int sk_scan_stream(sk_ctx *c, const uint8_t *stream, uint64_t nbytes, uint32_t col)
{
    if (!c || (!stream && nbytes)) return SK_E_ARG;
    if (!c->d_keys) return sk_fail(c, SK_E_STATE, "no table loaded");
    if (!c->d_counts) return sk_fail(c, SK_E_STATE, "no count columns (a union's context needs sk_union_count_enable)");
    if (col >= c->ncols) return sk_fail(c, SK_E_ARG, "column %u out of range", col);
    SK_HIP(c, hipSetDevice(c->device));
    int rc = sk_stage_init(c);
    if (rc) return rc;
    uint64_t done = 0;
    while (done < nbytes) {
        const uint64_t lead = done ? SK_OVERLAP : 0;
        uint64_t take = nbytes - done;
        if (take > SK_STAGE_BYTES - lead) take = SK_STAGE_BYTES - lead;
        const int b = c->stage_next;
        c->stage_next = (b + 1) % SK_NSTAGE;
        SK_HIP(c, hipEventSynchronize(c->stage_done[b]));
        memcpy(c->h_stage[b], stream + done - lead, lead + take);
        SK_HIP(c, hipMemcpyAsync(c->d_stage[b], c->h_stage[b], lead + take, hipMemcpyHostToDevice, c->stream));
        rc = sk_launch_scan(c, c->d_stage[b], lead + take, lead, col);
        if (rc) return rc;
        SK_HIP(c, hipEventRecord(c->stage_done[b], c->stream));
        done += take;
    }
    return SK_OK;
}

extern "C" int sk_pinned_alloc(sk_ctx *c, void **p, uint64_t nbytes)
{
    if (!c || !p) return SK_E_ARG;
    const size_t want = (size_t)((nbytes ? nbytes : 16) + 4095u) & ~(size_t)4095u;
    pthread_mutex_lock(&c->pin_mu);
    for (sk_pin &q : c->pins)
        if (!q.used && q.n == want) { q.used = true; *p = q.p; pthread_mutex_unlock(&c->pin_mu); return SK_OK; }
    pthread_mutex_unlock(&c->pin_mu);
    if (hipSetDevice(c->device) != hipSuccess) return SK_E_HIP;
    void *m = NULL;
    bool registered = true;
    if (posix_memalign(&m, 4096, want) != 0) return SK_E_NOMEM;
    if (hipHostRegister(m, want, hipHostRegisterPortable | hipHostRegisterMapped) != hipSuccess) {
        free(m);
        m = NULL;
        registered = false;
        (void)hipGetLastError();
        if (hipHostMalloc(&m, want, hipHostMallocPortable) != hipSuccess) return sk_fail(c, SK_E_NOMEM, "no page-locked memory (%zu bytes)", want);
    }
    pthread_mutex_lock(&c->pin_mu);
    c->pins.push_back((sk_pin){m, want, true, registered});
    pthread_mutex_unlock(&c->pin_mu);
    *p = m;
    return SK_OK;
}

extern "C" int sk_pinned_free(sk_ctx *c, void *p)
{
    if (!c) return SK_E_ARG;
    if (!p) return SK_OK;
    if (hipSetDevice(c->device) != hipSuccess || hipStreamSynchronize(c->stream) != hipSuccess) return SK_E_HIP;
    int rc = SK_E_ARG;
    pthread_mutex_lock(&c->pin_mu);
    for (sk_pin &q : c->pins) if (q.p == p && q.used) { q.used = false; rc = SK_OK; break; }
    pthread_mutex_unlock(&c->pin_mu);
    return rc;
}

static int sk_scan_pinned_n(sk_ctx *const *cs, uint32_t n, const void *src, uint64_t nbytes, uint64_t copy_bytes, bool packed,
                            uint32_t col, uint64_t *ticket)
{
    sk_ctx *const c = cs[0];
    SK_HIP(c, hipSetDevice(c->device));
    int rc = sk_stage_init(c);
    if (rc) return rc;
    const uint64_t t = c->tickets++;
    hipEvent_t &ev = c->copied[t & 63u];
    if (!ev) SK_HIP(c, hipEventCreateWithFlags(&ev, hipEventDisableTiming | (getenv("SK_SYNC") ? hipEventBlockingSync : 0u)));
    else SK_HIP(c, hipEventSynchronize(ev));
    const int b = c->stage_next;
    c->stage_next = (b + 1) % SK_NSTAGE;
    SK_HIP(c, hipStreamWaitEvent(c->copy_stream, c->stage_done[b], 0));
    if (copy_bytes) SK_HIP(c, hipMemcpyAsync(c->d_stage[b], src, copy_bytes, hipMemcpyHostToDevice, c->copy_stream));
    SK_HIP(c, hipEventRecord(ev, c->copy_stream));
    const uint8_t *const d = c->d_stage[b];
    const void *const inv = packed ? d + ((nbytes + 15u) >> 4) * 4u : NULL;
    for (uint32_t i = 0; i < n; i++) {
        sk_ctx *const m = cs[i];
        SK_HIP(c, hipStreamWaitEvent(m->stream, ev, 0));
        rc = sk_launch_scan(m, d, nbytes, 0, col, NULL, inv);
        if (rc) return m == c ? rc : sk_fail(c, rc, "context %u: %s", i, m->err);
        if (m != c) {
            if (!m->read_done) SK_HIP(c, hipEventCreateWithFlags(&m->read_done, hipEventDisableTiming));
            SK_HIP(c, hipEventRecord(m->read_done, m->stream));
            SK_HIP(c, hipStreamWaitEvent(c->stream, m->read_done, 0));
        }
    }
    SK_HIP(c, hipEventRecord(c->stage_done[b], c->stream));
    *ticket = t;
    return SK_OK;
}

extern "C" int sk_scan_pinned(sk_ctx *c, const uint8_t *pinned, uint64_t nbytes, uint32_t col, uint64_t *ticket)
{
    if (!c || (!pinned && nbytes) || !ticket) return SK_E_ARG;
    if (!c->d_keys) return sk_fail(c, SK_E_STATE, "no table loaded");
    if (!c->d_counts) return sk_fail(c, SK_E_STATE, "no count columns (a union's context needs sk_union_count_enable)");
    if (col >= c->ncols) return sk_fail(c, SK_E_ARG, "column %u out of range", col);
    if (nbytes > SK_STAGE_BYTES - 64) return sk_fail(c, SK_E_ARG, "pinned batch larger than the staging buffer");
    return sk_scan_pinned_n(&c, 1, pinned, nbytes, nbytes, false, col, ticket);
}

extern "C" int sk_scan_pinned_packed(sk_ctx *c, const void *packed, uint64_t nbytes, uint32_t col, uint64_t *ticket)
{
    if (!c || (!packed && nbytes) || !ticket) return SK_E_ARG;
    if (!c->d_keys) return sk_fail(c, SK_E_STATE, "no table loaded");
    if (!c->d_counts) return sk_fail(c, SK_E_STATE, "no count columns (a union's context needs sk_union_count_enable)");
    if (col >= c->ncols) return sk_fail(c, SK_E_ARG, "column %u out of range", col);
    const uint64_t nch = (nbytes + 15u) >> 4;
    if (nch * 6u > SK_STAGE_BYTES) return sk_fail(c, SK_E_ARG, "packed batch larger than the staging buffer");
    return sk_scan_pinned_n(&c, 1, packed, nbytes, nch * 6u, true, col, ticket);
}

static int sk_many_check(sk_ctx *const *cs, uint32_t n, uint32_t col)
{
    sk_ctx *const c = cs[0];
    for (uint32_t i = 0; i < n; i++) {
        const sk_ctx *m = cs[i];
        if (!m) return sk_fail(c, SK_E_ARG, "context %u is NULL", i);
        if (m->device != c->device) return sk_fail(c, SK_E_ARG, "context %u is on device %d, context 0 on %d: one upload serves one device", i, m->device, c->device);
        if (!m->d_keys) return sk_fail(c, SK_E_STATE, "context %u: no table loaded", i);
        if (!m->d_counts) return sk_fail(c, SK_E_STATE, "context %u: no count columns (a union's context needs sk_union_count_enable)", i);
        if (col >= m->ncols) return sk_fail(c, SK_E_ARG, "context %u: column %u out of range", i, col);
    }
    return SK_OK;
}

extern "C" int sk_scan_pinned_many(sk_ctx *const *ctx, uint32_t n, const uint8_t *pinned, uint64_t nbytes, uint32_t col, uint64_t *ticket)
{
    if (!ctx || n < 1 || !ctx[0] || (!pinned && nbytes) || !ticket) return SK_E_ARG;
    int rc = sk_many_check(ctx, n, col);
    if (rc) return rc;
    if (nbytes > SK_STAGE_BYTES - 64) return sk_fail(ctx[0], SK_E_ARG, "pinned batch larger than the staging buffer");
    return sk_scan_pinned_n(ctx, n, pinned, nbytes, nbytes, false, col, ticket);
}

extern "C" int sk_scan_pinned_packed_many(sk_ctx *const *ctx, uint32_t n, const void *packed, uint64_t nbytes, uint32_t col, uint64_t *ticket)
{
    if (!ctx || n < 1 || !ctx[0] || (!packed && nbytes) || !ticket) return SK_E_ARG;
    int rc = sk_many_check(ctx, n, col);
    if (rc) return rc;
    const uint64_t nch = (nbytes + 15u) >> 4;
    if (nch * 6u > SK_STAGE_BYTES) return sk_fail(ctx[0], SK_E_ARG, "packed batch larger than the staging buffer");
    return sk_scan_pinned_n(ctx, n, packed, nbytes, nch * 6u, true, col, ticket);
}

extern "C" int sk_device_memory(sk_ctx *c, uint64_t *free_bytes, uint64_t *total_bytes)
{
    if (!c || !free_bytes || !total_bytes) return SK_E_ARG;
    size_t f = 0, t = 0;
    SK_HIP(c, hipSetDevice(c->device));
    SK_HIP(c, hipMemGetInfo(&f, &t));
    *free_bytes = f; *total_bytes = t;
    return SK_OK;
}

extern "C" int sk_ticket_wait(sk_ctx *c, uint64_t ticket)
{
    if (!c || ticket >= c->tickets) return SK_E_ARG;
    if (c->tickets - ticket > 64) return SK_OK;
    SK_HIP(c, hipSetDevice(c->device));
    SK_HIP(c, hipEventSynchronize(c->copied[ticket & 63u]));
    return SK_OK;
}

extern "C" int sk_sync(sk_ctx *c)
{
    if (!c) return SK_E_ARG;
    SK_HIP(c, hipSetDevice(c->device));
    SK_HIP(c, hipStreamSynchronize(c->stream));
    return SK_OK;
}

extern "C" int sk_counts_fetch(sk_ctx *c, uint32_t col, uint32_t *out)
{
    if (!c || !out) return SK_E_ARG;
    if (!c->d_counts || col >= c->ncols) return sk_fail(c, SK_E_ARG, "bad column");
    SK_HIP(c, hipSetDevice(c->device));
    { int rc_ = sk_diff_flush(c); if (rc_) return rc_; }
    const uint32_t *src = c->d_counts + (size_t)col * c->nrows;
    if (c->d_perm && c->nrows) {
        hipLaunchKernelGGL(sk_gather_u32, dim3((c->nrows + 255) / 256), dim3(256), 0, c->stream, c->d_tmp, src, c->d_perm, c->nrows);
        src = c->d_tmp;
    }
    SK_HIP(c, hipMemcpyAsync(out, src, (size_t)c->nrows * 4, hipMemcpyDeviceToHost, c->stream));
    SK_HIP(c, hipStreamSynchronize(c->stream));
    return SK_OK;
}

extern "C" int sk_counts_set(sk_ctx *c, uint32_t col, const uint32_t *in)
{
    if (!c || !in) return SK_E_ARG;
    c->infbits_ok = false;
    if (!c->d_counts || col >= c->ncols) return sk_fail(c, SK_E_ARG, "bad column");
    SK_HIP(c, hipSetDevice(c->device));
    { int rc_ = sk_diff_flush(c); if (rc_) return rc_; }
    uint32_t *dst = c->d_counts + (size_t)col * c->nrows;
    if (c->d_perm && c->nrows) {
        SK_HIP(c, hipMemcpyAsync(c->d_tmp, in, (size_t)c->nrows * 4, hipMemcpyHostToDevice, c->stream));
        hipLaunchKernelGGL(sk_scatter_u32, dim3((c->nrows + 255) / 256), dim3(256), 0, c->stream, dst, c->d_tmp, c->d_perm, c->nrows);
    } else {
        SK_HIP(c, hipMemcpyAsync(dst, in, (size_t)c->nrows * 4, hipMemcpyHostToDevice, c->stream));
    }
    SK_HIP(c, hipStreamSynchronize(c->stream));
    return SK_OK;
}

extern "C" int sk_counts_set_rows(sk_ctx *c, uint32_t col, const uint32_t *rows, uint32_t n, uint32_t value)
{
    if (!c || (n && !rows)) return SK_E_ARG;
    c->infbits_ok = false;
    if (!c->d_counts || col >= c->ncols) return sk_fail(c, SK_E_ARG, "bad column");
    for (uint32_t i = 0; i < n; i++) if (rows[i] >= c->nrows) return sk_fail(c, SK_E_ARG, "row %u out of range", rows[i]);
    SK_HIP(c, hipSetDevice(c->device));
    { int rc_ = sk_diff_flush(c); if (rc_) return rc_; }
    if (!n) return SK_OK;
    uint32_t *d_rows = NULL;
    SK_HIP(c, hipMalloc((void **)&d_rows, (size_t)n * 4));
    hipError_t e = hipMemcpyAsync(d_rows, rows, (size_t)n * 4, hipMemcpyHostToDevice, c->stream);
    if (e == hipSuccess) {
        hipLaunchKernelGGL(sk_set_rows_u32, dim3((n + 255) / 256), dim3(256), 0, c->stream, c->d_counts + (size_t)col * c->nrows, (const uint32_t *)d_rows, n,
                           (const uint32_t *)c->d_perm, value);
        e = hipStreamSynchronize(c->stream);
    }
    (void)hipFree(d_rows);
    SK_HIP(c, e);
    return SK_OK;
}

extern "C" int sk_counts_zero(sk_ctx *c, uint32_t col)
{
    if (!c) return SK_E_ARG;
    c->infbits_ok = false;
    if (!c->d_counts || col >= c->ncols) return sk_fail(c, SK_E_ARG, "bad column");
    SK_HIP(c, hipSetDevice(c->device));
    { int rc_ = sk_diff_flush(c); if (rc_) return rc_; }
    SK_HIP(c, hipMemsetAsync(c->d_counts + (size_t)col * c->nrows, 0, (size_t)c->nrows * 4, c->stream));
    return SK_OK;
}

extern "C" void *sk_counts_device_ptr(sk_ctx *c)
{
    if (!c) return NULL;
    if (hipSetDevice(c->device) != hipSuccess || sk_diff_flush(c) != SK_OK || hipStreamSynchronize(c->stream) != hipSuccess) return NULL;
    return (void *)c->d_counts;
}

extern "C" int sk_fail_(sk_ctx *c, int code, const char *fmt, ...)
{
    if (c) {
        va_list ap;
        va_start(ap, fmt);
        vsnprintf(c->err, sizeof c->err, fmt, ap);
        va_end(ap);
    }
    return code;
}
extern "C" int sk_ctx_device_(const sk_ctx *c) { return c->device; }
extern "C" int sk_counts_rows_to_device_(sk_ctx *c, uint32_t col, uint32_t *d_out)
{
    if (!c || !d_out) return SK_E_ARG;
    if (!c->d_counts || col >= c->ncols) return sk_fail(c, SK_E_ARG, "bad column");
    SK_HIP(c, hipSetDevice(c->device));
    { int rc_ = sk_diff_flush(c); if (rc_) return rc_; }
    const uint32_t *src = c->d_counts + (size_t)col * c->nrows;
    if (c->d_perm && c->nrows)
        hipLaunchKernelGGL(sk_gather_u32, dim3((c->nrows + 255) / 256), dim3(256), 0, c->stream, d_out, src, c->d_perm, c->nrows);
    else
        SK_HIP(c, hipMemcpyAsync(d_out, src, (size_t)c->nrows * 4, hipMemcpyDeviceToDevice, c->stream));
    SK_HIP(c, hipStreamSynchronize(c->stream));
    return SK_OK;
}
extern "C" uint32_t sk_table_rows(const sk_ctx *c) { return c ? c->nrows : 0; }
extern "C" uint32_t sk_table_cols(const sk_ctx *c) { return c ? c->ncols : 0; }

extern "C" int sk_scan_timing(sk_ctx *c, double *total_ms, uint64_t *launches, int reset)
{
    if (!c) return SK_E_ARG;
    SK_HIP(c, hipSetDevice(c->device));
    SK_HIP(c, hipStreamSynchronize(c->stream));
    for (size_t i = 0; i + 1 < c->ev.size(); i += 2) {
        float ms = 0.f;
        SK_HIP(c, hipEventElapsedTime(&ms, c->ev[i], c->ev[i + 1]));
        c->timed_ms += ms;
        c->timed_launches++;
        c->ev_free.push_back(c->ev[i]);
        c->ev_free.push_back(c->ev[i + 1]);
    }
    c->ev.clear();
    if (total_ms) *total_ms = c->timed_ms;
    if (launches) *launches = c->timed_launches;
    if (reset) { c->timed_ms = 0; c->timed_launches = 0; }
    return SK_OK;
}

typedef struct { char internal[128]; } sk_nccl_id;
typedef int (*sk_nccl_allreduce_fn)(const void *, void *, size_t, int, int, void *, hipStream_t);
typedef int (*sk_nccl_getid_fn)(sk_nccl_id *);
typedef int (*sk_nccl_initrank_fn)(void **, int, sk_nccl_id, int);
typedef int (*sk_nccl_destroy_fn)(void *);
static struct { void *lib; sk_nccl_allreduce_fn allreduce; sk_nccl_getid_fn getid; sk_nccl_initrank_fn initrank; sk_nccl_destroy_fn destroy; } g_rccl;

static int sk_rccl_load(sk_ctx *c)
{
    if (g_rccl.lib) return SK_OK;
    void *h = dlopen("librccl.so.1", RTLD_NOW | RTLD_GLOBAL);
    if (!h) h = dlopen("librccl.so", RTLD_NOW | RTLD_GLOBAL);
    if (!h) return sk_fail(c, SK_E_RCCL, "cannot load librccl: %s", dlerror());
    g_rccl.allreduce = (sk_nccl_allreduce_fn)dlsym(h, "ncclAllReduce");
    g_rccl.getid = (sk_nccl_getid_fn)dlsym(h, "ncclGetUniqueId");
    g_rccl.initrank = (sk_nccl_initrank_fn)dlsym(h, "ncclCommInitRank");
    g_rccl.destroy = (sk_nccl_destroy_fn)dlsym(h, "ncclCommDestroy");
    if (!g_rccl.allreduce || !g_rccl.getid || !g_rccl.initrank || !g_rccl.destroy) return sk_fail(c, SK_E_RCCL, "RCCL symbols missing");
    g_rccl.lib = h;
    return SK_OK;
}

struct sk_watchdog { pthread_mutex_t mu; pthread_cond_t cv; int done; int timeout_s; int rank; };
static void *sk_watchdog_main(void *arg)
{
    sk_watchdog *w = (sk_watchdog *)arg;
    struct timespec until;
    clock_gettime(CLOCK_REALTIME, &until);
    until.tv_sec += w->timeout_s;
    pthread_mutex_lock(&w->mu);
    while (!w->done) {
        if (pthread_cond_timedwait(&w->cv, &w->mu, &until) == ETIMEDOUT && !w->done) {
            fprintf(stderr, "sk_comm_init: ncclCommInitRank did not return within %d s on rank %d (did a rank die after the rendezvous?) -- giving up\n",
                    w->timeout_s, w->rank);
            fflush(stderr);
            _exit(3);
        }
    }
    pthread_mutex_unlock(&w->mu);
    return NULL;
}

extern "C" int sk_comm_init_ex(sk_ctx *c, int rank, int world, const char *id_file, int timeout_s, int setup_failed)
{
    if (world < 1 || world > SKR_MAX_WORLD || rank < 0 || rank >= world || !id_file || (!c && !setup_failed)) return SK_E_ARG;
    if (timeout_s < 1) timeout_s = 1;
    sk_nccl_id id;
    memset(&id, 0, sizeof id);
    int failed = setup_failed != 0;
    if (!failed && sk_rccl_load(c) != SK_OK) failed = 1;
    if (!failed && hipSetDevice(c->device) != hipSuccess) failed = 1;
    if (!failed && rank == 0 && g_rccl.getid(&id) != 0) { sk_fail(c, SK_E_RCCL, "ncclGetUniqueId failed"); failed = 1; }
    static_assert(sizeof id == SKR_PAYLOAD, "RCCL unique id size");
    const int x = skr_exchange(rank, world, id_file, failed, (unsigned char *)&id, (double)timeout_s);
    if (rank == 0) {
    }
    if (x == SKR_ABORT) return sk_fail(c, SK_E_RCCL, failed ? "set-up failed on this rank; the other ranks were told to leave"
                                                            : "another rank reported a failed set-up: leaving before the collective");
    if (x == SKR_TIMEOUT) return sk_fail(c, SK_E_RCCL, "rendezvous through %s timed out after %d s (rank %d of %d)", id_file, timeout_s, rank, world);
    if (x != SKR_OK) return sk_fail(c, SK_E_RCCL, "rendezvous through %s failed (cannot write there?)", id_file);
    sk_watchdog w;
    pthread_mutex_init(&w.mu, NULL); pthread_cond_init(&w.cv, NULL);
    w.done = 0; w.timeout_s = timeout_s; w.rank = rank;
    pthread_t th;
    const bool watched = pthread_create(&th, NULL, sk_watchdog_main, &w) == 0;
    void *comm = NULL;
    const int nrc = g_rccl.initrank(&comm, world, id, rank);
    if (watched) {
        pthread_mutex_lock(&w.mu); w.done = 1; pthread_cond_signal(&w.cv); pthread_mutex_unlock(&w.mu);
        pthread_join(th, NULL);
    }
    pthread_mutex_destroy(&w.mu); pthread_cond_destroy(&w.cv);
    if (nrc != 0) return sk_fail(c, SK_E_RCCL, "ncclCommInitRank failed (rank %d of %d)", rank, world);
    c->comm = comm;
    c->comm_rank = rank;
    c->comm_world = world;
    return SK_OK;
}

extern "C" int sk_comm_init(sk_ctx *c, int rank, int world, const char *id_file, int timeout_s)
{
    if (!c) return SK_E_ARG;
    return sk_comm_init_ex(c, rank, world, id_file, timeout_s, 0);
}

extern "C" void sk_comm_destroy(sk_ctx *c)
{
    if (c && c->comm && g_rccl.destroy) { g_rccl.destroy(c->comm); c->comm = NULL; }
}

extern "C" int sk_comm_sum_u32(sk_ctx *c, uint32_t value, uint32_t *sum)
{
    if (!c || !sum) return SK_E_ARG;
    if (!c->comm) { *sum = value; return SK_OK; }
    SK_HIP(c, hipSetDevice(c->device));
    uint32_t *d = c->d_flags + 12;
    SK_HIP(c, hipMemcpyAsync(d, &value, 4, hipMemcpyHostToDevice, c->stream));
    const int ncclUint32 = 3, ncclSum = 0;
    if (g_rccl.allreduce(d, d, 1, ncclUint32, ncclSum, c->comm, c->stream) != 0) return sk_fail(c, SK_E_RCCL, "ncclAllReduce failed");
    SK_HIP(c, hipMemcpyAsync(sum, d, 4, hipMemcpyDeviceToHost, c->stream));
    SK_HIP(c, hipStreamSynchronize(c->stream));
    return SK_OK;
}

extern "C" int sk_comm_max_u64(sk_ctx *c, uint64_t *vals, uint32_t n)
{
    if (!vals || n == 0 || n > 8) return SK_E_ARG;
    if (!c || !c->comm) return SK_OK;
    SK_HIP(c, hipSetDevice(c->device));
    uint64_t *d = (uint64_t *)(c->d_flags + 16);
    SK_HIP(c, hipMemcpyAsync(d, vals, 8u * n, hipMemcpyHostToDevice, c->stream));
    const int ncclUint64 = 5, ncclMax = 2;
    if (g_rccl.allreduce(d, d, n, ncclUint64, ncclMax, c->comm, c->stream) != 0) return sk_fail(c, SK_E_RCCL, "ncclAllReduce failed");
    SK_HIP(c, hipMemcpyAsync(vals, d, 8u * n, hipMemcpyDeviceToHost, c->stream));
    SK_HIP(c, hipStreamSynchronize(c->stream));
    return SK_OK;
}

extern "C" int sk_comm_world(const sk_ctx *c) { return c && c->comm ? c->comm_world : 0; }

extern "C" int sk_comm_agree_u64(sk_ctx *c, uint64_t value, int *agree)
{
    if (!agree) return SK_E_ARG;
    *agree = 1;
    uint64_t h[2] = {value, ~value};
    const int rc = sk_comm_max_u64(c, h, 2);
    if (rc != SK_OK) return rc;
    *agree = h[0] == value && h[1] == ~value;
    return SK_OK;
}

extern "C" int sk_counts_allreduce(sk_ctx *c, void *rccl_comm)
{
    if (!c) return SK_E_ARG;
    if (!c->d_counts) return sk_fail(c, SK_E_STATE, "no table loaded");
    if (!rccl_comm) rccl_comm = c->comm;
    if (!rccl_comm) return sk_fail(c, SK_E_STATE, "no communicator");
    int rc = sk_rccl_load(c);
    if (rc) return rc;
    SK_HIP(c, hipSetDevice(c->device));
    if ((rc = sk_diff_flush(c)) != SK_OK) return rc;
    const int ncclUint32 = 3, ncclSum = 0;
    if (g_rccl.allreduce(c->d_counts, c->d_counts, (size_t)c->nrows * c->ncols, ncclUint32, ncclSum, rccl_comm, c->stream) != 0)
        return sk_fail(c, SK_E_RCCL, "ncclAllReduce failed");
    SK_HIP(c, hipStreamSynchronize(c->stream));
    return SK_OK;
}

extern "C" int sk_dev_alloc(sk_ctx *c, void **dev, uint64_t nbytes)
{
    if (!c || !dev) return SK_E_ARG;
    SK_HIP(c, hipSetDevice(c->device));
    if (c->dev_uncached) SK_HIP(c, hipExtMallocWithFlags(dev, nbytes ? nbytes : 16, hipDeviceMallocUncached));
    else SK_HIP(c, hipMalloc(dev, nbytes ? nbytes : 16));
    return SK_OK;
}

extern "C" int sk_dev_free(sk_ctx *c, void *dev)
{
    if (!c) return SK_E_ARG;
    SK_HIP(c, hipSetDevice(c->device));
    SK_HIP(c, hipStreamSynchronize(c->stream));
    SK_HIP(c, hipFree(dev));
    return SK_OK;
}

extern "C" int sk_dev_upload(sk_ctx *c, void *dev, const void *host, uint64_t nbytes)
{
    if (!c || !dev || !host) return SK_E_ARG;
    SK_HIP(c, hipSetDevice(c->device));
    SK_HIP(c, hipMemcpyAsync(dev, host, nbytes, hipMemcpyHostToDevice, c->stream));
    SK_HIP(c, hipStreamSynchronize(c->stream));
    return SK_OK;
}

extern "C" int sk_dev_download(sk_ctx *c, void *host, const void *dev, uint64_t nbytes)
{
    if (!c || !dev || !host) return SK_E_ARG;
    SK_HIP(c, hipSetDevice(c->device));
    SK_HIP(c, hipMemcpyAsync(host, dev, nbytes, hipMemcpyDeviceToHost, c->stream));
    SK_HIP(c, hipStreamSynchronize(c->stream));
    return SK_OK;
}

#if SK_PHASE_CLOCK
extern "C" int sk_debug_phase_clock(sk_ctx *c, unsigned long long out[8])
{
    if (!c || !out) return SK_E_ARG;
    SK_HIP(c, hipSetDevice(c->device));
    SK_HIP(c, hipStreamSynchronize(c->stream));
    unsigned long long *d = (unsigned long long *)(c->d_oddlist + (c->odd_cap ? c->odd_cap : SK_ODDCAP) - 1024u), h[512];
    SK_HIP(c, hipMemcpy(h, d, sizeof h, hipMemcpyDeviceToHost));
    SK_HIP(c, hipMemset(d, 0, sizeof h));
    for (int k = 0; k < 8; k++) { out[k] = 0; for (int s = 0; s < 64; s++) out[k] += h[s * 8 + k]; }
    return SK_OK;
}
#endif
```

Measured before the change: 2407 billion.

## Alternate device scans across two streams with per-lane flags and oddlists

Device-resident scans now alternate between two streams (lanes), each with its own flag block and odd-position list, so consecutive scan launches can overlap on the GPU. The wide-key kernel now resets its own flags using a last-block atomic counter, replacing the double-buffered next_flags scheme. A join is added before any operation that touches the main stream, and timing is changed to merge overlapping busy intervals across lanes. The cost is extra synchronisation logic, a second oddlist allocation, and a grid-wide atomic at the end of each wide kernel.

```diff
diff --git a/strainer2_amd/csrc/sk_dev_kernels.hip.h b/strainer2_amd/csrc/sk_dev_kernels.hip.h
--- a/strainer2_amd/csrc/sk_dev_kernels.hip.h
+++ b/strainer2_amd/csrc/sk_dev_kernels.hip.h
@@ -13,9 +13,8 @@
 __global__ __launch_bounds__(256)
 void sk_scan_wide(const uint8_t *__restrict__ stream, uint64_t nbytes, uint64_t emit_begin,
                   sk_table_view table, sk_wide_view wide, sk_sink sink,
-                  const uint32_t *__restrict__ flags, uint32_t *__restrict__ next_flags)
-{
-    if (blockIdx.x == 0u && threadIdx.x < 4u) next_flags[threadIdx.x] = 0u;
+                  uint32_t *flags)
+{
     if (flags[0] == 0u) return;
     const uint32_t nodd = flags[2];
     const bool listed = nodd <= table.oddcap;
@@ -72,6 +71,15 @@
             }
         }
     }
+    __syncthreads();
+    if (threadIdx.x == 0u) {
+        __threadfence();
+        if (atomicAdd(&flags[1], 1u) == gridDim.x - 1u) {
+            flags[0] = 0u; flags[2] = 0u; flags[3] = 0u;
+            __threadfence();
+            flags[1] = 0u;
+        }
+    }
 }
 
 __global__ void sk_fill64(uint64_t *p, uint64_t n, uint64_t v)
diff --git a/strainer2_amd/csrc/sk_device.hip b/strainer2_amd/csrc/sk_device.hip
--- a/strainer2_amd/csrc/sk_device.hip
+++ b/strainer2_amd/csrc/sk_device.hip
@@ -7,6 +7,7 @@
 #include <new>
 #include <string>
 #include <vector>
+#include <algorithm>
 #include <unistd.h>
 #include <pthread.h>
 #include <errno.h>
@@ -25,6 +26,16 @@
 #define SK_NSTAGE        2
 
 struct sk_pin { void *p; size_t n; bool used; bool registered; };
+#define SK_LANES 2
+struct sk_span { double b, e; };
+struct sk_lane {
+    hipStream_t  stream;
+    uint32_t    *d_flags;
+    uint32_t    *d_oddlist;
+    bool         flags_ready;
+    std::vector<hipEvent_t> ev;
+    std::vector<uint64_t> seq;
+};
 
 struct sk_ctx {
     int          device;
@@ -66,13 +77,18 @@
     hipEvent_t   read_done;
     uint64_t     tickets;
     uint32_t    *d_flags;
-    uint32_t     flag_set;
-    bool         flags_ready;
-    uint32_t    *d_oddlist;
-    std::vector<hipEvent_t> ev;
+    sk_lane      lane[SK_LANES];
+    long         scan_lanes;
+    uint32_t     lane_next;
+    bool         lane1_busy;
+    bool         lane1_behind;
+    hipEvent_t   lane_done, lane_go;
     std::vector<hipEvent_t> ev_free;
+    hipEvent_t   ev_base;
+    std::vector<sk_span> busy;
     double       timed_ms;
     uint64_t     timed_launches;
+    uint64_t     launch_seq;
     long         table_load_pct;
     long         ablate;
     long         dev_uncached;
@@ -155,8 +171,19 @@
     c->err[0] = 0;
     if (hipStreamCreateWithFlags(&c->stream, hipStreamNonBlocking) != hipSuccess) { delete c; return SK_E_NODEVICE; }
     if (hipMalloc((void **)&c->d_flags, 32 * sizeof(uint32_t)) != hipSuccess) { delete c; return SK_E_NOMEM; }
-    if (hipMalloc((void **)&c->d_oddlist, (size_t)SK_ODDCAP * sizeof(uint32_t)) != hipSuccess) { hipFree(c->d_flags); delete c; return SK_E_NOMEM; }
+    if (hipMalloc((void **)&c->lane[0].d_oddlist, (size_t)SK_ODDCAP * sizeof(uint32_t)) != hipSuccess) { hipFree(c->d_flags); delete c; return SK_E_NOMEM; }
     hipMemsetAsync(c->d_flags, 0, 32 * sizeof(uint32_t), c->stream);
+    c->lane[0].stream = c->stream;
+    for (uint32_t l = 0; l < SK_LANES; l++) c->lane[l].d_flags = c->d_flags + 4u * l;
+    c->scan_lanes = SK_LANES;
+    {
+        const char *e = getenv("SK_SCAN_LANES");
+        if (e && !strcmp(e, "1")) c->scan_lanes = 1;
+    }
+    c->lane1_behind = true;
+    if (hipEventCreate(&c->ev_base) != hipSuccess || hipEventRecord(c->ev_base, c->stream) != hipSuccess) {
+        hipFree(c->d_flags); hipFree(c->lane[0].d_oddlist); hipStreamDestroy(c->stream); delete c; return SK_E_NODEVICE;
+    }
     {
         static pthread_mutex_t once_mu = PTHREAD_MUTEX_INITIALIZER;
         static unsigned long long done_mask[4];
@@ -173,6 +200,75 @@
         if (e != hipSuccess) { delete c; return SK_E_NODEVICE; }
     }
     *out = c;
+    return SK_OK;
+}
+
+static int sk_lanes_join(sk_ctx *c)
+{
+    c->lane1_behind = true;
+    if (!c->lane1_busy) return SK_OK;
+    SK_HIP(c, hipEventRecord(c->lane_done, c->lane[1].stream));
+    SK_HIP(c, hipStreamWaitEvent(c->stream, c->lane_done, 0));
+    c->lane1_busy = false;
+    return SK_OK;
+}
+
+static int sk_lane1_init(sk_ctx *c)
+{
+    sk_lane &L = c->lane[1];
+    if (L.stream) return SK_OK;
+    if (!L.d_oddlist) SK_HIP(c, hipMalloc((void **)&L.d_oddlist, (size_t)SK_ODDCAP * sizeof(uint32_t)));
+    if (!c->lane_done) SK_HIP(c, hipEventCreateWithFlags(&c->lane_done, hipEventDisableTiming));
+    if (!c->lane_go) SK_HIP(c, hipEventCreateWithFlags(&c->lane_go, hipEventDisableTiming));
+    SK_HIP(c, hipStreamCreateWithFlags(&L.stream, hipStreamNonBlocking));
+    L.flags_ready = false;
+    return SK_OK;
+}
+
+#define SK_BUSY_KEEP 16u
+static void sk_timing_merge(sk_ctx *c, double b, double e)
+{
+    double add = e - b, mb = b, me = e;
+    std::vector<sk_span> keep;
+    for (const sk_span &s : c->busy) {
+        if (s.e < b || s.b > e) { keep.push_back(s); continue; }
+        add -= (e < s.e ? e : s.e) - (b > s.b ? b : s.b);
+        if (s.b < mb) mb = s.b;
+        if (s.e > me) me = s.e;
+    }
+    if (add > 0.0) c->timed_ms += add;
+    size_t at = keep.size();
+    while (at > 0 && keep[at - 1].b > mb) at--;
+    keep.insert(keep.begin() + at, (sk_span){mb, me});
+    if (keep.size() > SK_BUSY_KEEP) keep.erase(keep.begin(), keep.end() - SK_BUSY_KEEP);
+    c->busy.swap(keep);
+}
+static void sk_timing_rebase(sk_ctx *c, hipEvent_t &e0, double at)
+{
+    std::swap(c->ev_base, e0);
+    for (sk_span &s : c->busy) { s.b -= at; s.e -= at; }
+}
+static int sk_timing_add(sk_ctx *c, hipEvent_t &e0, hipEvent_t e1)
+{
+    float ms = 0.f, at = 0.f;
+    SK_HIP(c, hipEventElapsedTime(&ms, e0, e1));
+    c->timed_launches++;
+    if (!c->lane[1].stream) { c->timed_ms += ms; return SK_OK; }
+    SK_HIP(c, hipEventElapsedTime(&at, c->ev_base, e0));
+    sk_timing_merge(c, (double)at, (double)at + (double)ms);
+    if (at > 1000.f) sk_timing_rebase(c, e0, (double)at);
+    return SK_OK;
+}
+
+static int sk_timing_retire(sk_ctx *c, sk_lane &L)
+{
+    SK_HIP(c, hipEventSynchronize(L.ev[1]));
+    int trc = sk_timing_add(c, L.ev[0], L.ev[1]);
+    if (trc) return trc;
+    c->ev_free.push_back(L.ev[0]);
+    c->ev_free.push_back(L.ev[1]);
+    L.ev.erase(L.ev.begin(), L.ev.begin() + 2);
+    L.seq.erase(L.seq.begin());
     return SK_OK;
 }
 
@@ -210,7 +306,9 @@
 {
     if (!c) return;
     hipSetDevice(c->device);
+    (void)sk_lanes_join(c);
     hipStreamSynchronize(c->stream);
+    if (c->lane[1].stream) { hipStreamSynchronize(c->lane[1].stream); hipStreamDestroy(c->lane[1].stream); }
     sk_comm_destroy(c);
     sk_table_release(c);
     for (int i = 0; i < SK_NSTAGE; i++) {
@@ -219,8 +317,11 @@
         if (c->stage_done[i]) hipEventDestroy(c->stage_done[i]);
     }
     if (c->copy_stream) { hipStreamSynchronize(c->copy_stream); hipStreamDestroy(c->copy_stream); }
-    for (hipEvent_t e : c->ev) hipEventDestroy(e);
+    for (sk_lane &L : c->lane) for (hipEvent_t e : L.ev) hipEventDestroy(e);
     for (hipEvent_t e : c->ev_free) hipEventDestroy(e);
+    if (c->ev_base) hipEventDestroy(c->ev_base);
+    if (c->lane_done) hipEventDestroy(c->lane_done);
+    if (c->lane_go) hipEventDestroy(c->lane_go);
     for (int i = 0; i < 64; i++) if (c->copied[i]) hipEventDestroy(c->copied[i]);
     if (c->read_done) hipEventDestroy(c->read_done);
     if (c->own_batch) sk_batch_destroy(c->own_batch);
@@ -230,7 +331,7 @@
     for (sk_pin &q : c->pins) { if (q.registered) { hipHostUnregister(q.p); free(q.p); } else hipHostFree(q.p); }
     pthread_mutex_destroy(&c->pin_mu);
     hipFree(c->d_flags);
-    hipFree(c->d_oddlist);
+    for (sk_lane &L : c->lane) hipFree(L.d_oddlist);
     hipStreamDestroy(c->stream);
     delete c;
 }
@@ -244,6 +345,13 @@
     if (!strcmp(name, "dev_alloc_uncached")) { c->dev_uncached = value != 0; return SK_OK; }
     if (!strcmp(name, "text_stage")) { c->no_text = value == 0; return SK_OK; }
     if (!strcmp(name, "pipeline")) { if (value < 0 || value > 2) return SK_E_ARG; c->pipeline = value; return SK_OK; }
+    if (!strcmp(name, "scan_lanes")) {
+        if (value < 1 || value > SK_LANES) return SK_E_ARG;
+        if (value == 1 && c->lane1_busy) { SK_HIP(c, hipSetDevice(c->device)); int rc = sk_lanes_join(c); if (rc) return rc; }
+        c->scan_lanes = value;
+        c->lane_next = 0;
+        return SK_OK;
+    }
 #ifdef SK_EXPERIMENTS
     if (!strcmp(name, "ablate")) { c->ablate = value; return SK_OK; }
 #else
@@ -269,6 +377,7 @@
         }
     }
     SK_HIP(c, hipSetDevice(c->device));
+    { int jrc = sk_lanes_join(c); if (jrc) return jrc; }
     SK_HIP(c, hipStreamSynchronize(c->stream));
     sk_table_release(c);
 
@@ -282,7 +391,7 @@
     SK_HIP(c, hipMemsetAsync(c->d_counts, 0, cbytes, c->stream));
     hipLaunchKernelGGL(sk_fill64, dim3(2048), dim3(256), 0, c->stream, (uint64_t *)c->d_keys, 2 * slots, SK_EMPTY64);
     SK_HIP(c, hipMemsetAsync(c->d_flags, 0, 16 * sizeof(uint32_t), c->stream));
-    c->flags_ready = false;
+    for (sk_lane &L : c->lane) L.flags_ready = false;
     if (nrows) {
         uint64_t *d_in = NULL;
         SK_HIP(c, hipMalloc((void **)&d_in, (size_t)nrows * sizeof(uint64_t)));
@@ -384,6 +493,7 @@
     uint32_t run = 0;
     for (size_t b = 0; b < nblk; b++) { rank[b].x = run; run += (uint32_t)__builtin_popcount(rank[b].y) + (uint32_t)__builtin_popcount(rank[b].z); }
     SK_HIP(c, hipSetDevice(c->device));
+    { int jrc = sk_lanes_join(c); if (jrc) return jrc; }
     SK_HIP(c, hipStreamSynchronize(c->stream));
     hipFree(c->d_text2); c->d_text2 = NULL;
     hipFree(c->d_rank); c->d_rank = NULL;
@@ -422,6 +532,7 @@
     if (!c || !text2 || !startok || !nrows_out || ncols == 0 || ncols > 16) return SK_E_ARG;
     if (nbases < SK_K || nbases > 0x7FFFFF00u) return sk_fail(c, SK_E_ARG, "text of %u bases (a table slot holds 31 bits of position)", nbases);
     SK_HIP(c, hipSetDevice(c->device));
+    { int jrc = sk_lanes_join(c); if (jrc) return jrc; }
     SK_HIP(c, hipStreamSynchronize(c->stream));
     sk_table_release(c);
     uint32_t *d_ok = NULL;
@@ -454,7 +565,7 @@
     SK_HIP(c, hipMemsetAsync(c->d_text2, 0, words * 4, c->stream));
     SK_HIP(c, hipMemsetAsync(c->d_rank, 0, nblk * sizeof(sk_u4), c->stream));
     SK_HIP(c, hipMemsetAsync(c->d_flags, 0, 16 * sizeof(uint32_t), c->stream));
-    c->flags_ready = false;
+    for (sk_lane &L : c->lane) L.flags_ready = false;
     SK_HIP(c, hipMemcpyAsync(c->d_text2, text2, have * 4, hipMemcpyHostToDevice, c->stream));
     SK_HIP(c, hipMemcpyAsync(d_ok, startok, bwords * 4, hipMemcpyHostToDevice, c->stream));
     const dim3 grid((nbases + 255) / 256), block(256);
@@ -523,6 +634,7 @@
     if (!c->d_keys_by_row) return sk_fail(c, SK_E_STATE, "no key list to export (sk_table_build_from_text first)");
     for (uint32_t i = 0; i < n; i++) if (rows[i] >= c->nrows) return sk_fail(c, SK_E_ARG, "row %u out of range", rows[i]);
     SK_HIP(c, hipSetDevice(c->device));
+    { int jrc = sk_lanes_join(c); if (jrc) return jrc; }
     void *d = NULL;
     SK_HIP(c, hipMalloc(&d, (size_t)n * 12));
     uint64_t *d_out = (uint64_t *)d;
@@ -550,6 +662,7 @@
 
 static int sk_diff_flush(sk_ctx *c)
 {
+    { int jrc = sk_lanes_join(c); if (jrc) return jrc; }
     if (c->diff_col < 0 || !c->d_diff) { c->diff_col = -1; return SK_OK; }
     const uint32_t n = c->nrows + 1u, nb = (n + SK_DIFF_PER_BLOCK - 1u) / SK_DIFF_PER_BLOCK;
     hipLaunchKernelGGL(sk_diff_block_sums, dim3(nb), dim3(256), 0, c->stream, c->d_diff, n, c->d_diff_sums);
@@ -564,7 +677,7 @@
 static int sk_scratch(sk_ctx *c, void **p, size_t *cap, size_t need);
 
 static int sk_launch_scan(sk_ctx *c, const uint8_t *d_stream, uint64_t nbytes, uint64_t emit_begin, uint32_t col,
-                          const sk_sink *tally_sink = NULL, const void *packed_inv = NULL)
+                          const sk_sink *tally_sink = NULL, const void *packed_inv = NULL, bool lane_scan = false)
 {
     if (nbytes <= emit_begin || c->nrows == 0) return SK_OK;
     const uint64_t ntiles = (nbytes + SK_TILE - 1) / SK_TILE;
@@ -573,7 +686,7 @@
     tv.nrows = c->nrows;
     tv.text2 = c->no_text ? NULL : c->d_text2; tv.rank = c->d_rank; tv.text_bases = c->text_bases;
     tv.slots = c->d_keys; tv.mask = (uint32_t)(((uint64_t)1 << c->slots_log2) - 1);
-    tv.oddlist = c->d_oddlist; tv.oddcap = c->odd_cap ? (uint32_t)c->odd_cap : SK_ODDCAP;
+    tv.oddcap = c->odd_cap ? (uint32_t)c->odd_cap : SK_ODDCAP;
     tv.grid1 = c->d_grid1; tv.grid2 = c->d_grid2;
     tv.grid1_blocks = c->grid1_blocks; tv.grid2_shift = 32u - c->grid2_blocks_log2;
     sk_wide_view wv;
@@ -594,25 +707,41 @@
     }
     const dim3 grid((uint32_t)ntiles), block(SK_THREADS);
     if (!c->d_grid1) return sk_fail(c, SK_E_STATE, "no table loaded");
+    uint32_t li = 0;
+    if (lane_scan && !tally_sink && c->scan_lanes > 1 && !c->ablate && c->pipeline != 2 && !SK_PHASE_CLOCK) {
+        if (c->grid_pending) { int jrc = sk_lanes_join(c); if (jrc) return jrc; }
+        li = c->lane_next;
+        c->lane_next ^= 1u;
+    } else {
+        int jrc = sk_lanes_join(c);
+        if (jrc) return jrc;
+    }
     { int grc = sk_grid_ensure(c); if (grc) return grc; }
-
-    if (!c->flags_ready) {
-        SK_HIP(c, hipMemsetAsync(c->d_flags, 0, 8 * sizeof(uint32_t), c->stream));
-        c->flags_ready = true;
-    }
-    c->flag_set ^= 1u;
-    uint32_t *const d_fl = c->d_flags + 4u * c->flag_set, *const d_fl_next = c->d_flags + 4u * (c->flag_set ^ 1u);
+    if (li) {
+        int lrc = sk_lane1_init(c);
+        if (lrc) return lrc;
+        if (c->lane1_behind) {
+            SK_HIP(c, hipEventRecord(c->lane_go, c->stream));
+            SK_HIP(c, hipStreamWaitEvent(c->lane[1].stream, c->lane_go, 0));
+            c->lane1_behind = false;
+        }
+        c->lane1_busy = true;
+    }
+    sk_lane &L = c->lane[li];
+    const hipStream_t st = L.stream;
+    tv.oddlist = L.d_oddlist;
+    if (!L.flags_ready) {
+        SK_HIP(c, hipMemsetAsync(L.d_flags, 0, 4 * sizeof(uint32_t), st));
+        L.flags_ready = true;
+    }
+    uint32_t *const d_fl = L.d_flags;
     hipEvent_t e0 = NULL, e1 = NULL;
     const bool timed = true;
-    if (c->ev.size() >= 2 * SK_EV_PAIRS) {
-        float ms = 0.f;
-        SK_HIP(c, hipEventSynchronize(c->ev[1]));
-        SK_HIP(c, hipEventElapsedTime(&ms, c->ev[0], c->ev[1]));
-        c->timed_ms += ms;
-        c->timed_launches++;
-        c->ev_free.push_back(c->ev[0]);
-        c->ev_free.push_back(c->ev[1]);
-        c->ev.erase(c->ev.begin(), c->ev.begin() + 2);
+    if (L.ev.size() >= 2 * SK_EV_PAIRS) {
+        sk_lane &O = c->lane[li ^ 1u];
+        while (!O.seq.empty() && O.seq[0] < L.seq[0]) { int trc = sk_timing_retire(c, O); if (trc) return trc; }
+        int trc = sk_timing_retire(c, L);
+        if (trc) return trc;
     }
     if (c->ev_free.size() >= 2) {
         e1 = c->ev_free.back(); c->ev_free.pop_back();
@@ -621,15 +750,15 @@
         SK_HIP(c, hipEventCreate(&e0));
         SK_HIP(c, hipEventCreate(&e1));
     }
-    SK_HIP(c, hipEventRecord(e0, c->stream));
+    SK_HIP(c, hipEventRecord(e0, st));
     const bool piped = !packed_inv && (!c->ablate || c->ablate >= 7) && c->pipeline == 2;
     const uint8_t *d_cand = NULL;
     if (piped && !c->d_grid3) {
         const size_t b3 = (size_t)SK_BIN_P * SK_BIN_WORDS * 4;
         const uint64_t nslots = (uint64_t)1 << c->slots_log2;
         SK_HIP(c, hipMalloc((void **)&c->d_grid3, b3));
-        SK_HIP(c, hipMemsetAsync(c->d_grid3, 0, b3, c->stream));
-        hipLaunchKernelGGL(sk_grid3_insert, dim3((uint32_t)((nslots + 255) / 256)), dim3(256), 0, c->stream, (const sk_u4 *)c->d_keys, nslots, c->d_grid3);
+        SK_HIP(c, hipMemsetAsync(c->d_grid3, 0, b3, st));
+        hipLaunchKernelGGL(sk_grid3_insert, dim3((uint32_t)((nslots + 255) / 256)), dim3(256), 0, st, (const sk_u4 *)c->d_keys, nslots, c->d_grid3);
     }
     if (piped) {
         const uint64_t ntiles_bin = (nbytes + SK_BIN_TILE - 1) / SK_BIN_TILE;
@@ -637,8 +766,8 @@
         if ((rc = sk_scratch(c, &c->p_bins, &c->p_bins_cap, (size_t)ntiles_bin * SK_BIN_P * SK_BIN_CAP * 4)) != SK_OK) return rc;
         if ((rc = sk_scratch(c, &c->p_binn, &c->p_binn_cap, (size_t)ntiles_bin * SK_BIN_P)) != SK_OK) return rc;
         if ((rc = sk_scratch(c, &c->p_cand, &c->p_cand_cap, (size_t)ntiles_bin * SK_BIN_CH + 64)) != SK_OK) return rc;
-        SK_HIP(c, hipMemsetAsync(c->p_cand, 0, (size_t)ntiles_bin * SK_BIN_CH + 64, c->stream));
-        hipLaunchKernelGGL(sk_bin, dim3((uint32_t)ntiles_bin), dim3(256), 0, c->stream, d_stream, nbytes, tv,
+        SK_HIP(c, hipMemsetAsync(c->p_cand, 0, (size_t)ntiles_bin * SK_BIN_CH + 64, st));
+        hipLaunchKernelGGL(sk_bin, dim3((uint32_t)ntiles_bin), dim3(256), 0, st, d_stream, nbytes, tv,
                            (uint32_t *)c->p_bins, (uint8_t *)c->p_binn, (uint32_t)ntiles_bin, (uint8_t *)c->p_cand, d_fl);
         uint32_t splits = ntiles_bin >= 4096 ? 4u : ntiles_bin >= 1024 ? 2u : 1u;
         static bool lds_attr = false;
@@ -646,23 +775,23 @@
             SK_HIP(c, hipFuncSetAttribute((const void *)sk_lds_probe, hipFuncAttributeMaxDynamicSharedMemorySize, (int)(SK_BIN_WORDS * 4)));
             lds_attr = true;
         }
-        hipLaunchKernelGGL(sk_lds_probe, dim3(SK_BIN_P * splits), dim3(1024), SK_BIN_WORDS * 4, c->stream, (const uint32_t *)c->d_grid3,
+        hipLaunchKernelGGL(sk_lds_probe, dim3(SK_BIN_P * splits), dim3(1024), SK_BIN_WORDS * 4, st, (const uint32_t *)c->d_grid3,
                            (const uint32_t *)c->p_bins, (const uint8_t *)c->p_binn, (uint32_t)ntiles_bin, splits, (uint8_t *)c->p_cand);
         d_cand = (const uint8_t *)c->p_cand;
     }
-#define SK_LAUNCH_GRID(T, A, C) hipLaunchKernelGGL((sk_scan_grid<T, A, C>), grid, block, 0, c->stream, \
+#define SK_LAUNCH_GRID(T, A, C) hipLaunchKernelGGL((sk_scan_grid<T, A, C>), grid, block, 0, st, \
                                                    d_stream, nbytes, emit_begin, tv, sink, d_fl, d_cand)
     if (packed_inv) {
         if (c->ablate) return sk_fail(c, SK_E_UNSUPPORTED, "no ablations on packed batches");
         if (tally_sink && tally_sink->ns)
-            hipLaunchKernelGGL((sk_scan_grid<true, 0, false, true, true>), grid, block, 0, c->stream, d_stream, nbytes, emit_begin, tv, sink, d_fl, (const uint8_t *)packed_inv);
+            hipLaunchKernelGGL((sk_scan_grid<true, 0, false, true, true>), grid, block, 0, st, d_stream, nbytes, emit_begin, tv, sink, d_fl, (const uint8_t *)packed_inv);
         else if (tally_sink)
-            hipLaunchKernelGGL((sk_scan_grid<true, 0, false, false, true>), grid, block, 0, c->stream, d_stream, nbytes, emit_begin, tv, sink, d_fl, (const uint8_t *)packed_inv);
+            hipLaunchKernelGGL((sk_scan_grid<true, 0, false, false, true>), grid, block, 0, st, d_stream, nbytes, emit_begin, tv, sink, d_fl, (const uint8_t *)packed_inv);
         else
-            hipLaunchKernelGGL((sk_scan_grid<false, 0, false, false, true>), grid, block, 0, c->stream, d_stream, nbytes, emit_begin, tv, sink, d_fl, (const uint8_t *)packed_inv);
+            hipLaunchKernelGGL((sk_scan_grid<false, 0, false, false, true>), grid, block, 0, st, d_stream, nbytes, emit_begin, tv, sink, d_fl, (const uint8_t *)packed_inv);
     }
     else if (tally_sink && tally_sink->ns)
-        hipLaunchKernelGGL((sk_scan_grid<true, 0, false, true>), grid, block, 0, c->stream, d_stream, nbytes, emit_begin, tv, sink, d_fl, d_cand);
+        hipLaunchKernelGGL((sk_scan_grid<true, 0, false, true>), grid, block, 0, st, d_stream, nbytes, emit_begin, tv, sink, d_fl, d_cand);
     else if (piped && tally_sink) SK_LAUNCH_GRID(true, 0, true);
 #ifdef SK_EXPERIMENTS
     else if (piped && c->ablate == 7) SK_LAUNCH_GRID(false, 7, true);
@@ -683,22 +812,23 @@
     else                     SK_LAUNCH_GRID(false, 0, false);
 #undef SK_LAUNCH_GRID
     if (timed) {
-        SK_HIP(c, hipEventRecord(e1, c->stream));
-        c->ev.push_back(e0);
-        c->ev.push_back(e1);
+        SK_HIP(c, hipEventRecord(e1, st));
+        L.ev.push_back(e0);
+        L.ev.push_back(e1);
+        L.seq.push_back(c->launch_seq++);
     }
     uint64_t wblocks = (nbytes - emit_begin + 255) / 256;
     if (wblocks > 2048) wblocks = 2048;
     if (wblocks == 0) { wblocks = 1; }
     if (tally_sink && tally_sink->ns)
-        hipLaunchKernelGGL((sk_scan_wide<true, true>), dim3((uint32_t)wblocks), dim3(256), 0, c->stream,
-                           d_stream, nbytes, emit_begin, tv, wv, sink, d_fl, d_fl_next);
+        hipLaunchKernelGGL((sk_scan_wide<true, true>), dim3((uint32_t)wblocks), dim3(256), 0, st,
+                           d_stream, nbytes, emit_begin, tv, wv, sink, d_fl);
     else if (tally_sink)
-        hipLaunchKernelGGL(sk_scan_wide<true>, dim3((uint32_t)wblocks), dim3(256), 0, c->stream,
-                           d_stream, nbytes, emit_begin, tv, wv, sink, d_fl, d_fl_next);
+        hipLaunchKernelGGL(sk_scan_wide<true>, dim3((uint32_t)wblocks), dim3(256), 0, st,
+                           d_stream, nbytes, emit_begin, tv, wv, sink, d_fl);
     else
-        hipLaunchKernelGGL(sk_scan_wide<false>, dim3((uint32_t)wblocks), dim3(256), 0, c->stream,
-                           d_stream, nbytes, emit_begin, tv, wv, sink, d_fl, d_fl_next);
+        hipLaunchKernelGGL(sk_scan_wide<false>, dim3((uint32_t)wblocks), dim3(256), 0, st,
+                           d_stream, nbytes, emit_begin, tv, wv, sink, d_fl);
     SK_HIP(c, hipGetLastError());
     return SK_OK;
 }
@@ -1166,6 +1296,7 @@
     if (!u) return SK_E_ARG;
     sk_ctx *c = u->uc;
     SK_HIP(c, hipSetDevice(c->device));
+    { int jrc = sk_lanes_join(c); if (jrc) return jrc; }
     SK_HIP(c, hipStreamSynchronize(c->stream));
     c->t_inflight_nrec = 0;
     return SK_OK;
@@ -1249,7 +1380,7 @@
     if (col >= c->ncols) return sk_fail(c, SK_E_ARG, "column %u out of range", col);
     if (((uintptr_t)dev_stream & 15u) != 0) return sk_fail(c, SK_E_ARG, "device stream must be 16-byte aligned");
     SK_HIP(c, hipSetDevice(c->device));
-    return sk_launch_scan(c, (const uint8_t *)dev_stream, nbytes, 0, col);
+    return sk_launch_scan(c, (const uint8_t *)dev_stream, nbytes, 0, col, NULL, NULL, true);
 }
 
 extern "C" int sk_scan_device_packed(sk_ctx *c, const void *dev_packed, uint64_t nbytes, uint32_t col)
@@ -1261,7 +1392,7 @@
     if (((uintptr_t)dev_packed & 3u) != 0) return sk_fail(c, SK_E_ARG, "device batch must be 4-byte aligned");
     SK_HIP(c, hipSetDevice(c->device));
     const uint64_t nch = (nbytes + 15u) >> 4;
-    return sk_launch_scan(c, (const uint8_t *)dev_packed, nbytes, 0, col, NULL, (const uint8_t *)dev_packed + nch * 4u);
+    return sk_launch_scan(c, (const uint8_t *)dev_packed, nbytes, 0, col, NULL, (const uint8_t *)dev_packed + nch * 4u, true);
 }
 
 static int sk_stage_init(sk_ctx *c)
@@ -1333,7 +1464,7 @@
 {
     if (!c) return SK_E_ARG;
     if (!p) return SK_OK;
-    if (hipSetDevice(c->device) != hipSuccess || hipStreamSynchronize(c->stream) != hipSuccess) return SK_E_HIP;
+    if (hipSetDevice(c->device) != hipSuccess || sk_lanes_join(c) != SK_OK || hipStreamSynchronize(c->stream) != hipSuccess) return SK_E_HIP;
     int rc = SK_E_ARG;
     pthread_mutex_lock(&c->pin_mu);
     for (sk_pin &q : c->pins) if (q.p == p && q.used) { q.used = false; rc = SK_OK; break; }
@@ -1452,6 +1583,7 @@
 {
     if (!c) return SK_E_ARG;
     SK_HIP(c, hipSetDevice(c->device));
+    { int jrc = sk_lanes_join(c); if (jrc) return jrc; }
     SK_HIP(c, hipStreamSynchronize(c->stream));
     return SK_OK;
 }
@@ -1562,16 +1694,26 @@
 {
     if (!c) return SK_E_ARG;
     SK_HIP(c, hipSetDevice(c->device));
-    SK_HIP(c, hipStreamSynchronize(c->stream));
-    for (size_t i = 0; i + 1 < c->ev.size(); i += 2) {
-        float ms = 0.f;
-        SK_HIP(c, hipEventElapsedTime(&ms, c->ev[i], c->ev[i + 1]));
-        c->timed_ms += ms;
-        c->timed_launches++;
-        c->ev_free.push_back(c->ev[i]);
-        c->ev_free.push_back(c->ev[i + 1]);
-    }
-    c->ev.clear();
+    { int jrc = sk_lanes_join(c); if (jrc) return jrc; }
+    SK_HIP(c, hipStreamSynchronize(c->stream));
+    if (!c->lane[1].stream) {
+        for (size_t i = 0; i + 1 < c->lane[0].ev.size(); i += 2) { int trc = sk_timing_add(c, c->lane[0].ev[i], c->lane[0].ev[i + 1]); if (trc) return trc; }
+    } else {
+        struct span { double b, e; hipEvent_t *e0; };
+        std::vector<span> sp;
+        for (sk_lane &L : c->lane)
+            for (size_t i = 0; i + 1 < L.ev.size(); i += 2) {
+                float ms = 0.f, at = 0.f;
+                SK_HIP(c, hipEventElapsedTime(&ms, L.ev[i], L.ev[i + 1]));
+                SK_HIP(c, hipEventElapsedTime(&at, c->ev_base, L.ev[i]));
+                sp.push_back((span){(double)at, (double)at + (double)ms, &L.ev[i]});
+            }
+        std::sort(sp.begin(), sp.end(), [](const span &x, const span &y) { return x.b < y.b; });
+        for (const span &x : sp) { sk_timing_merge(c, x.b, x.e); c->timed_launches++; }
+        if (!sp.empty() && sp.back().b > 1000.0) sk_timing_rebase(c, *sp.back().e0, sp.back().b);
+    }
+    for (sk_lane &L : c->lane) { c->ev_free.insert(c->ev_free.end(), L.ev.begin(), L.ev.end()); }
+    for (sk_lane &L : c->lane) { L.ev.clear(); L.seq.clear(); }
     if (total_ms) *total_ms = c->timed_ms;
     if (launches) *launches = c->timed_launches;
     if (reset) { c->timed_ms = 0; c->timed_launches = 0; }
@@ -1739,6 +1881,7 @@
 {
     if (!c) return SK_E_ARG;
     SK_HIP(c, hipSetDevice(c->device));
+    { int jrc = sk_lanes_join(c); if (jrc) return jrc; }
     SK_HIP(c, hipStreamSynchronize(c->stream));
     SK_HIP(c, hipFree(dev));
     return SK_OK;
@@ -1748,6 +1891,7 @@
 {
     if (!c || !dev || !host) return SK_E_ARG;
     SK_HIP(c, hipSetDevice(c->device));
+    { int jrc = sk_lanes_join(c); if (jrc) return jrc; }
     SK_HIP(c, hipMemcpyAsync(dev, host, nbytes, hipMemcpyHostToDevice, c->stream));
     SK_HIP(c, hipStreamSynchronize(c->stream));
     return SK_OK;
@@ -1757,6 +1901,7 @@
 {
     if (!c || !dev || !host) return SK_E_ARG;
     SK_HIP(c, hipSetDevice(c->device));
+    { int jrc = sk_lanes_join(c); if (jrc) return jrc; }
     SK_HIP(c, hipMemcpyAsync(host, dev, nbytes, hipMemcpyDeviceToHost, c->stream));
     SK_HIP(c, hipStreamSynchronize(c->stream));
     return SK_OK;
@@ -1767,8 +1912,9 @@
 {
     if (!c || !out) return SK_E_ARG;
     SK_HIP(c, hipSetDevice(c->device));
-    SK_HIP(c, hipStreamSynchronize(c->stream));
-    unsigned long long *d = (unsigned long long *)(c->d_oddlist + (c->odd_cap ? c->odd_cap : SK_ODDCAP) - 1024u), h[512];
+    { int jrc = sk_lanes_join(c); if (jrc) return jrc; }
+    SK_HIP(c, hipStreamSynchronize(c->stream));
+    unsigned long long *d = (unsigned long long *)(c->lane[0].d_oddlist + (c->odd_cap ? c->odd_cap : SK_ODDCAP) - 1024u), h[512];
     SK_HIP(c, hipMemcpy(h, d, sizeof h, hipMemcpyDeviceToHost));
     SK_HIP(c, hipMemset(d, 0, sizeof h));
     for (int k = 0; k < 8; k++) { out[k] = 0; for (int s = 0; s < 64; s++) out[k] += h[s * 8 + k]; }
```

Result: faster. 2463 billion, median of 6 (+2.4%).
